# amankhullar/MMBiDAF

Measured on NVIDIA B200. Metric: mmbidaf_train_videos_per_s, higher is better.
Workload: dtype bf16 tcgen05 BiDAF + tf32 library GEMMs, fp32 accumulate / soft-max / LSTM

## Files before the change

### include/mmbidaf_b200.h

```cpp
#ifndef MMBIDAF_B200_H_
#define MMBIDAF_B200_H_

#include <stddef.h>
#include <stdint.h>

#ifdef __cplusplus
extern "C" {
#endif

#if defined(__GNUC__)
#define MMB_API __attribute__((visibility("default")))
#else
#define MMB_API
#endif

typedef void* mmb_stream_t;

enum mmb_status {
  MMB_OK = 0,
  MMB_ERR_INVALID = 1,
  MMB_ERR_UNSUPPORTED = 2,
  MMB_ERR_CUDA = 3
};

// ... 82 lines not shown
                                               const float* out_wt, const float* out_b, const float* emb_text, const float* h0,
                                               const uint8_t* mask, const int32_t* text_len, long long* tokens, int32_t* parents,
                                               float* scores, float* probs, long long* best, int32_t* path, int B, int Lt, int D, int H,
                                               int E, int M, int K, int S, int no_repeat, int min_sentences, mmb_stream_t stream);
MMB_API int mmb_decoder_beam_sample_fused(const float* proj_a, const float* proj_i, const float* enc_a, const float* enc_i,
                                          const float* Wh4t, const float* bh4, const float* v1, const float* wc1, const float* v2,
                                          const float* wc2, const float* v1b, const float* v2b, const float* Wb13t, const float* vb1,
                                          const float* vb2, const float* vb1b, const float* vb2b, const float* Wcatt, const float* bcat,
                                          const float* out_wt, const float* out_b, const float* emb_text, const float* h0,
                                          const uint8_t* mask, const int32_t* text_len, const unsigned long long* key, long long* tokens,
                                          int32_t* parents, float* scores, float* probs, float* phi, float* keys, long long* paths,
                                          int32_t* path_slots, float* kappa, int B, int Lt, int D, int H, int E, int M, int K, int S,
                                          float T, int no_repeat, int min_sentences, mmb_stream_t stream);
MMB_API int mmb_decoder_sample_fused(const float* proj_a, const float* proj_i, const float* enc_a, const float* enc_i,
                                     const float* Wh4t, const float* bh4, const float* v1, const float* wc1, const float* v2,
                                     const float* wc2, const float* v1b, const float* v2b, const float* Wb13t, const float* vb1,
                                     const float* vb2, const float* vb1b, const float* vb2b, const float* Wcatt, const float* bcat,
                                     const float* out_wt, const float* out_b, const float* emb_text, const float* h0,
                                     const uint8_t* mask, const int32_t* text_len, const unsigned long long* key, float* probs,
                                     long long* tokens, int B, int Lt, int D, int H, int E, int M, int S, int N, float T, int top_k,
                                     int no_repeat, int min_sentences, mmb_stream_t stream);
MMB_API int mmb_sample_pick(const float* probs, const uint8_t* eligible, const unsigned long long* key, const int32_t* row_base, int R,
                            int M, int S, int s, int N, float T, int top_k, long long* picks, mmb_stream_t stream);
MMB_API int mmb_decoder_sample_nucleus_fused(const float* proj_a, const float* proj_i, const float* enc_a, const float* enc_i,
                                             const float* Wh4t, const float* bh4, const float* v1, const float* wc1, const float* v2,
                                             const float* wc2, const float* v1b, const float* v2b, const float* Wb13t, const float* vb1,
                                             const float* vb2, const float* vb1b, const float* vb2b, const float* Wcatt, const float* bcat,
                                             const float* out_wt, const float* out_b, const float* emb_text, const float* h0,
                                             const uint8_t* mask, const int32_t* text_len, const unsigned long long* key, float* probs,
                                             long long* tokens, int B, int Lt, int D, int H, int E, int M, int S, int N, float T,
                                             int top_k, int no_repeat, int min_sentences, float top_p, mmb_stream_t stream);
MMB_API int mmb_sample_pick_nucleus(const float* probs, const uint8_t* eligible, const unsigned long long* key, const int32_t* row_base,
                                    int R, int M, int S, int s, int N, float T, int top_k, long long* picks, float top_p,
                                    mmb_stream_t stream);
MMB_API int mmb_greedy_select(const long long* argmax, const int32_t* text_len, int32_t* sel, int32_t* count, int B, int S,
                              mmb_stream_t stream);

MMB_API int mmb_decoder_attn_fwd(const float* proj_a, const float* proj_i, const float* enc_a, const float* enc_i,
                                 const float* hw, const float* coverage, const float* v1, const float* wc1,
                                 const float* v2, const float* wc2, const float* v1b, const float* v2b, float* p,
                                 float* stats, float* ctxp, float* ctx12, float* scale, int* counters, int B, int Lt, int D,
                                 int nch, mmb_stream_t stream);
MMB_API int mmb_decoder_attn_finish(const float* pb, const float* hw, const float* ctx12, const float* scale,
                                    const float* coverage, const float* sent, const float* h, const float* vb1,
                                    const float* vb2, const float* vb1b, const float* vb2b, float* p_alpha, float* xcat,
                                    float* att_cov, float* cov_out, float* beta, float* cov_loss, int B, int Lt, int D,
                                    int E, int H, int nch, mmb_stream_t stream);
MMB_API int mmb_decoder_cell_fwd(float* gates, const float* cell, float* h_out, float* cell_out, int B, int H,
                                 mmb_stream_t stream);
MMB_API int mmb_decoder_out_softmax(float* logits, const uint8_t* mask, long long* argmax, const long long* target,
                                    float* nll, int B, int M, mmb_stream_t stream);

MMB_API int mmb_decoder_bwd_head(const float* probs, const float* d_probs, const long long* target, const float* g_nll,
                                 const float* g_cov, const float* out_w, const float* gates, const float* cell_in,
                                 const float* cell_out, const float* d_h_out, const float* d_cell_out, const float* Wcat_ctx,
                                 const float* d_att_cov, const float* d_cov_out, const float* alpha, const float* beta,
                                 const float* ctx12, const float* pb, const float* hw, const float* vb1, const float* vb2,
                                 const float* att, const float* cov_out, const float* Wb13, float* d_logits, int ldd, float* d_gates,
                                 int ldg, float* d_cell, float* datt, float* dcov_tot, float* d_pre_b, float* d_ctx12, float* vec_acc,
                                 float* scal_acc, int B, int Lt, int D, int H, int M, mmb_stream_t stream);
MMB_API int mmb_decoder_out_softmax_bwd(const float* probs, const float* d_probs, const long long* target,
                                        const float* g_nll, float* d_logits, int ldd, int B, int M, mmb_stream_t stream);
MMB_API int mmb_decoder_cell_bwd(float* gates, const float* cell_in, const float* cell_out, const float* d_h,
                                 const float* d_h2, const float* d_cell_out, float* d_gates, int ldg, float* d_cell,
                                 int B, int H, mmb_stream_t stream);
MMB_API int mmb_decoder_attn_finish_bwd(const float* d_xcat, int ldx, const float* d_att_cov, const float* d_cov_out,
                                        const float* alpha, const float* beta, const float* ctx12, const float* pb,
                                        const float* hw, const float* vb1, const float* vb2, float* datt, float* d_pre_b,
                                        float* d_ctx12, float* vec_acc, float* scal_acc, const float* att_cov,
                                        const float* cov_out, const float* g_cov, float* dcov_tot, int B, int Lt, int D,
                                        mmb_stream_t stream);
MMB_API int mmb_decoder_step_fused_bwd(const float* probs, const float* d_probs, const long long* target, const float* g_nll,
                                       const float* g_cov, const float* out_w, const float* gates, const float* cell_in,
                                       const float* cell_out, const float* d_h_out, const float* d_cell_out, const float* Wcat_ctx,
                                       const float* d_att_cov, const float* d_cov_out, const float* alpha, const float* beta,
                                       const float* ctx12, const float* pb, const float* hw, const float* vb1, const float* vb2,
                                       const float* att, const float* cov_out, const float* Wb13, float* d_logits, int ldd,
                                       float* d_gates, int ldg, float* d_cell, float* datt, float* dcov_tot, float* d_pre_b,
                                       float* d_ctx12, float* vec_acc, float* scal_acc, const float* proj_a, const float* proj_i,
                                       const float* enc_a, const float* enc_i, const float* coverage, const float* v1, const float* wc1,
                                       const float* v2, const float* wc2, float* d_proj_a, float* d_proj_i, float* d_cov,
                                       const float* Wh_stack, float* d_h, int B, int Lt, int D, int H, int M, mmb_stream_t stream);

MMB_API int mmb_decoder_attn_bwd(const float* proj_a, const float* proj_i, const float* enc_a, const float* enc_i,
                                 const float* hw, const float* coverage, const float* alpha, const float* beta,
                                 const float* datt, const float* d_ctx12, const float* d_cov_out, const float* d_pre_b,
                                 const float* v1, const float* wc1, const float* v2, const float* wc2, float* d_alpha,
                                 float* spart, float* d_proj_a, float* d_proj_i, float* d_cov, float* colp, float* separt,
                                 float* d_hw4, int ldhw, float* vec_acc, float* scal_acc, int* counters, int B, int Lt,
                                 int D, int nch, mmb_stream_t stream);

MMB_API int mmb_masked_softmax_fwd(const float* x, const uint8_t* mask, float* y, long long rows, int n, int log_mode,
                                   mmb_stream_t stream);
MMB_API int mmb_masked_softmax_bwd(const float* y, const float* dy, const uint8_t* mask, float* dx, long long rows,
                                   int n, int log_mode, mmb_stream_t stream);

MMB_API int mmb_highway_fwd(const float* pre, const float* x, float* y, long long n, int H, mmb_stream_t stream);
MMB_API int mmb_highway_bwd(const float* pre, const float* x, const float* dy, float* d_pre, float* dx_direct,
                            long long n, int H, mmb_stream_t stream);

MMB_API int mmb_length_plan(const int32_t* lengths, uint8_t* mask, uint8_t* dec_mask, int32_t* order, int B, int L, int M,
                            mmb_stream_t stream);

MMB_API int mmb_col_sum_blocks(long long n, int p);
MMB_API int mmb_col_sum(const float* a, float* partial, float* out, long long n, int p, mmb_stream_t stream);

MMB_API int mmb_pack_segments(const float* const* srcs, const long long* dst_offsets, const long long* sizes, int n_segs, float* dst,
                              mmb_stream_t stream);

MMB_API int mmb_adadelta_clip_step(float* param, float* grad, float* square_avg, float* acc_delta, const float* grad_norm,
                                   float max_norm, float lr, float rho, float eps, float weight_decay, long long n,
                                   mmb_stream_t stream);

#ifdef __cplusplus
}
#endif
#endif
```

### mmbidaf_b200/_lib.py

```python
from __future__ import annotations

import ctypes
import os
from typing import Optional

import torch

_PKG = os.path.dirname(os.path.abspath(__file__))
LIB_PATH = os.path.join(_PKG, "libmmbidaf_b200.so")

_lib: Optional[ctypes.CDLL] = None
_device_ok = False

c_void_p, c_int, c_float, c_size_t = ctypes.c_void_p, ctypes.c_int, ctypes.c_float, ctypes.c_size_t

SIGNATURES = {
    "mmb_version": [],
    "mmb_last_error": [],
    "mmb_device_supported": [],
    "mmb_bidaf_fwd": [c_void_p] * 10 + [c_float] + [c_void_p] * 6 + [c_int] * 5 + [c_void_p],
    "mmb_bidaf_workspace_bytes": [c_int] * 6,
    "mmb_bidaf_bwd": [c_void_p] * 11 + [c_float] + [c_void_p] * 13 + [c_int] * 5 + [c_void_p],
    "mmb_bidaf_bwd_workspace_bytes": [c_int] * 5,
    "mmb_bilstm_fwd": [c_void_p] * 8 + [c_int] * 5 + [c_void_p],
    "mmb_bilstm_bwd": [c_void_p] * 8 + [c_int] * 4 + [c_void_p],
    "mmb_bilstm_fwd_dropout": [c_void_p] * 10 + [c_float] + [c_int] * 5 + [c_void_p],
    "mmb_bilstm_bwd_dropout": [c_void_p] * 9 + [c_float] + [c_int] * 4 + [c_void_p],
    "mmb_dropout_mask": [c_void_p, c_float, ctypes.c_longlong, c_void_p, c_void_p],
    "mmb_rng_next": [c_void_p, c_void_p, c_int, c_void_p],
    "mmb_dropout_apply": [c_void_p, c_void_p, c_void_p, c_float, ctypes.c_longlong, c_void_p],
    "mmb_decoder_chunks": [c_int, c_int],
    "mmb_decoder_step_fused_fwd": [c_void_p] * 42 + [c_int] * 6 + [c_void_p],
    "mmb_decoder_greedy_fused": [c_void_p] * 28 + [c_int] * 8 + [c_void_p],
    "mmb_decoder_beam_fused": [c_void_p] * 31 + [c_int] * 8 + [c_void_p],
    "mmb_decoder_greedy_constrained_fused": [c_void_p] * 27 + [c_int] * 9 + [c_void_p],
    "mmb_decoder_beam_constrained_fused": [c_void_p] * 31 + [c_int] * 10 + [c_void_p],
    "mmb_decoder_beam_sample_fused": [c_void_p] * 35 + [c_int] * 8 + [c_float] + [c_int] * 2 + [c_void_p],
    "mmb_decoder_sample_fused":[c_void_p] * 28 + [c_int] * 8 + [c_float] + [c_int] * 3 + [c_void_p],
    "mmb_sample_pick": [c_void_p] * 4 + [c_int] * 5 + [c_float, c_int, c_void_p, c_void_p],
    "mmb_decoder_sample_nucleus_fused": [c_void_p] * 28 + [c_int] * 8 + [c_float] + [c_int] * 3 + [c_float, c_void_p],
    "mmb_sample_pick_nucleus": [c_void_p] * 4 + [c_int] * 5 + [c_float, c_int, c_void_p, c_float, c_void_p],
    "mmb_greedy_select": [c_void_p] * 4 + [c_int] * 2 + [c_void_p],
    "mmb_decoder_bwd_head": [c_void_p] * 25 + [c_int] + [c_void_p] + [c_int] + [c_void_p] * 7 + [c_int] * 5 + [c_void_p],
    "mmb_decoder_attn_fwd": [c_void_p] * 18 + [c_int] * 4 + [c_void_p],
    "mmb_decoder_attn_finish": [c_void_p] * 17 + [c_int] * 6 + [c_void_p],
    "mmb_decoder_cell_fwd": [c_void_p] * 4 + [c_int] * 2 + [c_void_p],
    "mmb_decoder_out_softmax": [c_void_p] * 5 + [c_int] * 2 + [c_void_p],
    "mmb_decoder_out_softmax_bwd": [c_void_p] * 5 + [c_int] * 3 + [c_void_p],
    "mmb_decoder_cell_bwd": [c_void_p] * 7 + [c_int] + [c_void_p] + [c_int] * 2 + [c_void_p],
    "mmb_decoder_attn_finish_bwd": [c_void_p, c_int] + [c_void_p] * 18 + [c_int] * 3 + [c_void_p],
    "mmb_decoder_step_fused_bwd": [c_void_p] * 25 + [c_int] + [c_void_p] + [c_int] + [c_void_p] * 21 + [c_int] * 5 + [c_void_p],
    "mmb_decoder_attn_bwd": [c_void_p] * 24 + [c_int] + [c_void_p] * 3 + [c_int] * 4 + [c_void_p],
    "mmb_highway_fwd": [c_void_p] * 3 + [ctypes.c_longlong, c_int, c_void_p],
    "mmb_highway_bwd": [c_void_p] * 5 + [ctypes.c_longlong, c_int, c_void_p],
    "mmb_length_plan": [c_void_p] * 4 + [c_int] * 3 + [c_void_p],
    "mmb_pack_segments": [c_void_p] * 3 + [c_int] + [c_void_p] * 2,
    "mmb_col_sum_blocks": [ctypes.c_longlong, c_int],
    "mmb_col_sum": [c_void_p] * 3 + [ctypes.c_longlong, c_int, c_void_p],
    "mmb_adadelta_clip_step": [c_void_p] * 5 + [c_float] * 5 + [ctypes.c_longlong, c_void_p],
    "mmb_masked_softmax_fwd": [c_void_p] * 3 + [ctypes.c_longlong, c_int, c_int, c_void_p],
    "mmb_masked_softmax_bwd": [c_void_p] * 4 + [ctypes.c_longlong, c_int, c_int, c_void_p],
}
_RESTYPES = {"mmb_last_error": ctypes.c_char_p, "mmb_bidaf_workspace_bytes": c_size_t,
             "mmb_bidaf_bwd_workspace_bytes": c_size_t}


DECODER_WEIGHT_FIELDS = ("W2", "b2", "Wc1", "bc1", "v1", "v1b", "W4", "b4", "Wc2", "bc2", "v2", "v2b",
                         "Wb1", "bb1", "Wb2", "bb2", "Wb3", "bb3", "Wb4", "bb4", "vb1", "vb1b", "vb2", "vb2b",
                         "lstm_w_ih", "lstm_w_hh", "lstm_b_ih", "lstm_b_hh", "out_w", "out_b")


def load() -> ctypes.CDLL:
    global _lib
    if _lib is None:
        if not os.path.exists(LIB_PATH):
            raise RuntimeError(f"{LIB_PATH} is missing: run `python -m mmbidaf_b200.build` "
                               "(there is no CPU or PyTorch fallback for the mmbidaf_b200 kernels)")
        lib = ctypes.CDLL(LIB_PATH)
        for name, argtypes in SIGNATURES.items():
            fn = getattr(lib, name)
            fn.argtypes = argtypes
            fn.restype = _RESTYPES.get(name, c_int)
        _lib = lib
    return _lib


def lib() -> ctypes.CDLL:
    global _device_ok
    handle = load()
    if not _device_ok:
        if not torch.cuda.is_available():
            raise RuntimeError("mmbidaf_b200 needs a CUDA device (sm_100a); none is visible and there is no CPU path")
        if not handle.mmb_device_supported():
            raise RuntimeError(handle.mmb_last_error().decode())
        _device_ok = True
    return handle


def check(status: int, what: str) -> None:
    if status != 0:
        raise RuntimeError(f"{what} failed (status {status}): {load().mmb_last_error().decode()}")


def ptr(t: Optional[torch.Tensor]) -> Optional[int]:
    if t is None:
        return None
    assert t.is_cuda and t.is_contiguous(), "mmbidaf_b200 ops take contiguous CUDA tensors"
    return t.data_ptr()


def stream() -> int:
    return torch.cuda.current_stream().cuda_stream
```

### mmbidaf_b200/csrc/decoder_fused.cu

```cuda
#include <cooperative_groups.h>
#include <stdlib.h>
#include <type_traits>
#include "common.cuh"
#include "tc_common.cuh"

namespace cg = cooperative_groups;

namespace mmb {
namespace {

constexpr int NT = 512;
constexpr int NW = NT / 32;
constexpr int MAXC = 8;
constexpr int SCR = 2048;
__host__ __device__ constexpr int split4(int n, int parts) { return ((n + parts - 1) / parts + 3) & ~3; }

__device__ __forceinline__ float rcp_ftz(float x) {
  float y;
  asm("rcp.approx.ftz.f32 %0, %1;" : "=f"(y) : "f"(x));
  return y;
}

__device__ __forceinline__ void bulk_reduce_add_f32(float* dst, uint32_t src_smem, uint32_t bytes) {
  asm volatile("cp.reduce.async.bulk.global.shared::cta.bulk_group.add.f32 [%0], [%1], %2;" ::"l"(dst), "r"(src_smem), "r"(bytes)
// ... 252 lines not shown
      const float p = m < M ? v[m] : -1.f;
      const uint32_t bits = __float_as_uint(p);
      uint32_t q = __float2uint_rz(p * 16777216.f);
      const bool in = q != 0u && (bits & pmask) == prefix;
      const uint32_t digit = in ? (bits >> shift) & (kNucBuckets - 1) : kNucBuckets;
      q = in ? q : 0u;
      const uint32_t peers = __match_any_sync(0xffffffffu, digit);
      const uint32_t sum = __reduce_add_sync(peers, q);
      if (in && lane == __ffs(peers) - 1) atomicAdd(hist + digit, (unsigned long long)sum);
    }
    __syncthreads();
    const unsigned long long h = tid < kNucBuckets ? hist[kNucBuckets - 1 - tid] : 0ull;
    unsigned long long s = h;
#pragma unroll
    for (int o = 1; o < 32; o <<= 1) {
      const unsigned long long t = __shfl_up_sync(0xffffffffu, s, o);
      if (lane >= o) s += t;
    }
    if (lane == 31 && warp < kNucBuckets / 32) red[warp] = s;
    __syncthreads();
    unsigned long long below = 0, total = 0;
    for (int w = 0; w < kNucBuckets / 32; ++w) {
      below += w < warp ? red[w] : 0ull;
      total += red[w];
    }
    s += below;
    if (pass == 0) {
      const unsigned long long pq = (unsigned long long)P * total;
      rem = (pq >> 24) + ((pq & 0xffffffull) != 0ull);
      if (rem == 0ull) { first = true; break; }
    }
    if (tid < kNucBuckets && s - h < rem && rem <= s) {
      red[8] = (unsigned long long)(kNucBuckets - 1 - tid);
      red[9] = rem - (s - h);
    }
    __syncthreads();
    prefix |= (uint32_t)red[8] << shift;
    pmask |= (uint32_t)(kNucBuckets - 1) << shift;
    rem = red[9];
  }
  unsigned long long ties = 1;
  if (first) {
    uint32_t mx = 0;
    for (int m = tid; m < M; m += NT) {
      const float p = v[m];
      if (p >= 0.f) mx = max(mx, __float_as_uint(p));
    }
    mx = __reduce_max_sync(0xffffffffu, mx);
    __syncthreads();
    if (lane == 0) red[warp] = mx;
    __syncthreads();
    prefix = 0;
    for (int w = 0; w < NW; ++w) prefix = max(prefix, (uint32_t)red[w]);
  } else {
    const unsigned long long qs = __float2uint_rz(__uint_as_float(prefix) * 16777216.f);
    ties = (rem + qs - 1) / qs;
  }
  const int c = (M + NT - 1) / NT, lo = min(M, tid * c), hi = min(M, lo + c);
  int cnt = 0;
  for (int m = lo; m < hi; ++m) cnt += __float_as_uint(v[m]) == prefix;
  int incl = cnt;
#pragma unroll
  for (int o = 1; o < 32; o <<= 1) {
    const int t = __shfl_up_sync(0xffffffffu, incl, o);
    if (lane >= o) incl += t;
  }
  __syncthreads();
  if (lane == 31) red[warp] = (unsigned long long)incl;
  if (tid == 0) red[NW] = ~0ull;
  __syncthreads();
  unsigned long long excl = (unsigned long long)(incl - cnt);
  for (int w = 0; w < warp; ++w) excl += red[w];
  if (excl < ties && ties <= excl + (unsigned long long)cnt) {
    unsigned long long k = excl;
    for (int m = lo; m < hi; ++m)
      if (__float_as_uint(v[m]) == prefix && ++k == ties) red[NW] = (unsigned long long)m;
  }
  __syncthreads();
  const NucleusCut cut{prefix, (int)(long long)red[NW]};
  __syncthreads();
  return cut;
}

template <bool kGreedy, bool kBeam = false, bool kConstrained = false, bool kSample = false, bool kNucleus = false, bool kStoch = false>
__device__ __forceinline__ void dec_fused_body(const FusedArgs& a, const GreedyArgs& g, const BeamArgs& bm, const ConstraintArgs& cn,
                                               const SampleArgs sp, const NucleusArgs nu = NucleusArgs{}, const StochArgs st = StochArgs{}) {
  cg::cluster_group cluster = cg::this_cluster();
  const int CL = (int)cluster.num_blocks(), R = (int)cluster.block_rank();
  const int ob = blockIdx.x / CL;
  const int b = kSample ? cluster_row() / sp.N : ob;
  const int tid = threadIdx.x, lane = tid & 31, warp = tid >> 5;
  const int D = a.D, H = a.H, E = a.E, M = a.M, Lt = a.Lt, K = D + E + H;

  extern __shared__ __align__(16) float smem[];
  auto up4 = [](int v) { return (v + 3) & ~3; };
  float* s_hw = smem;
  float* s_x = s_hw + up4(4 * D);
  float* s_ctx = s_x + up4(K);
  float* s_pb = s_ctx + up4(2 * D);
  float* s_hn = s_pb + up4(2 * D);
  float* s_part = s_hn + up4(H);
  float* s_ex = s_part + up4(MAXC * (4 + 2 * D));
  float* s_g = s_ex + MAXC * 8;
  float* s_red = s_g + up4(4 * (split4(H, MAXC / 2) + 1));
  float* s_scr = s_red + 32;
  float* s_vec = s_scr + SCR;
  float* s_e = s_vec + up4(4 * D);
  float* s_cov = s_e + up4(2 * a.chunk);
  float* s_cpart = s_cov + up4(a.chunk);

  const int t0 = min(Lt, R * a.chunk), t1 = min(Lt, t0 + a.chunk), n = t1 - t0;
  const bool staged = a.stage_off != 0;
  float* const s_st0 = smem + a.stage_off + 4;
  float* const s_st1 = s_st0 + up4(a.chunk * D);
  const uint32_t bar_proj = tc::smem_u32(smem + a.stage_off), bar_enc = bar_proj + 8;
  const uint32_t stage_bytes = (uint32_t)(n * D) * 4u;
  if (staged && tid == 0) {
    tc::mbar_init(bar_proj, 1);
    tc::mbar_init(bar_enc, 1);
    tc::fence_barrier_init();
    if (n > 0) {
      tc::mbar_expect_tx(bar_proj, 2 * stage_bytes, 1);
      tc::tma_bulk_g2s(tc::smem_u32(s_st0), a.proj_a + ((size_t)b * Lt + t0) * D, stage_bytes, bar_proj, 1);
      tc::tma_bulk_g2s(tc::smem_u32(s_st1), a.proj_i + ((size_t)b * Lt + t0) * D, stage_bytes, bar_proj, 1);
    }
  }
  DEC_STAMP(0);
  const int S = kGreedy ? g.steps : 1;
  float cell_own = 0.f;
  int pick = 0;
  const int KW = kBeam ? bm.K : 1;
  const int ldh = up4(H), ldc = up4(split4(H, CL)), ldv = up4(a.chunk), ldp = up4((M + CL - 1) / CL);
  float* const bs_score = smem + (kSample ? sp.off : bm.off);
  int* const bs_tok = reinterpret_cast<int*>(bs_score + MAXK);
  int* const bs_stat = bs_tok + MAXK;
  float* const nt_score = bs_score + 3 * MAXK;
  int* const nt_tok = reinterpret_cast<int*>(nt_score + MAXK);
  int* const nt_par = nt_tok + MAXK;
  int* const nt_kind = nt_par + MAXK;
  constexpr int CS = kStoch ? MAXK + 1 : MAXK;
  float* const s_cand = nt_score + 4 * MAXK;
  float* const s_wred = s_cand + MAXC * CS * 4;
  float* const s_loc = s_wred + NW * 4;
  float* const s_bh = s_loc + CS * 4;
  float* const s_bhn = s_bh + KW * ldh;
  float* const s_bc = s_bhn + KW * ldh;
  float* const s_bcn = s_bc + KW * ldc;
  float* const s_bcv = s_bcn + KW * ldc;
  float* const s_bcvn = s_bcv + KW * ldv;
  float* const s_bp = s_bcvn + KW * ldv;
  const int eos = kBeam ? bm.text_len[b] - 1 : kConstrained ? cn.text_len[b] - 1 : 0;
  int runs = 0;
  const int e_per = (M + CL - 1) / CL, e_m0 = min(M, R * e_per), e_m1 = min(M, e_m0 + e_per);
  auto allowed0 = [&](int m) { return m < e_m1 && m <= eos && a.mask[(size_t)b * M + m] != 0; };
  const int ldu = (ldp + 31) / 32;
  uint32_t* bu_cur = reinterpret_cast<uint32_t*>(s_bp + KW * ldp);
  uint32_t* bu_nxt = bu_cur + KW * ldu;
  int* bk_cur = reinterpret_cast<int*>(bu_nxt + KW * ldu);
  int* bk_nxt = bk_cur + MAXK;
  uint32_t allow = 0;
  int kept = 0;
  uint32_t key0 = 0, key1 = 0;
  float inv_t = 1.f;
  if constexpr (kSample && !kConstrained) {
    const unsigned long long key = *sp.key;
    key0 = (uint32_t)key;
    key1 = (uint32_t)(key >> 32);
// ... 271 lines not shown
      block_matvec_t(a.Wb13t + (size_t)k * D * D, D, nullptr, s_ctx + k * D, D, hi - lo, s_scr, SCR, ((lo - k * D) & 3) == 0,
                     [&](int i) { return lo - k * D + i; },
                     [&](int i, float v) {
                       const int o = lo + i;
                       for (int r = 0; r < CL; ++r) cluster.map_shared_rank(s_pb, r)[o] = v;
                       if constexpr (!kGreedy) a.pb[((size_t)k * a.B + b) * D + (o - k * D)] = v;
                     });
    }
  }
  DEC_STAMP(9);
  cluster.sync();
  DEC_STAMP(10);
  float beta1, beta2;
  {
    float eb1 = 0.f, eb2 = 0.f;
    for (int d = tid; d < D; d += NT) {
      eb1 = fmaf(a.vb1[d], tanh_fast(s_pb[d] + s_hw[2 * D + d]), eb1);
      eb2 = fmaf(a.vb2[d], tanh_fast(s_pb[D + d] + s_hw[3 * D + d]), eb2);
    }
    eb1 = block_sum(eb1, s_red) + a.vb1b[0];
    eb2 = block_sum(eb2, s_red) + a.vb2b[0];
    const float mb = fmaxf(eb1, eb2);
    const float x1 = expf(eb1 - mb), x2 = expf(eb2 - mb);
    beta1 = x1 / (x1 + x2);
    beta2 = x2 / (x1 + x2);
    for (int d = tid; d < D; d += NT) s_x[d] = s_ctx[d] * beta1 + s_ctx[D + d] * beta2;
    float closs = 0.f;
    for (int i = tid; i < n; i += NT) {
      const int t = t0 + i;
      const float a1 = s_e[i] * scale_own[0], a2 = s_e[a.chunk + i] * scale_own[1];
      if constexpr (!kGreedy) {
        a.alpha[((size_t)b * 2 + 0) * Lt + t] = a1;
        a.alpha[((size_t)b * 2 + 1) * Lt + t] = a2;
      }
      const float att = a1 * beta1 + a2 * beta2;
      if constexpr (kBeam) {
        const float cnew = s_cov[i] + att;
        s_bcvn[slot * ldv + i] = cnew;
        closs += fminf(att, cnew);
      } else if constexpr (kGreedy) {
        const float cnew = s_cov[i] + att;
        s_cov[i] = cnew;
        closs += fminf(att, cnew);
      } else {
        const float cnew = a.cov[(size_t)b * Lt + t] + att;
        a.att_cov[(size_t)b * Lt + t] = att;
        a.cov_out[(size_t)b * Lt + t] = cnew;
        closs += fminf(att, cnew);
      }
    }
    closs = block_sum(closs, s_red);
    if (tid == 0) cluster.map_shared_rank(s_ex, 0)[R * 8 + 0] = closs;
    if (!kGreedy && R == 0 && tid == 0) {
      a.beta[b * 2 + 0] = beta1;
      a.beta[b * 2 + 1] = beta2;
    }
  }
  __syncthreads();
  if (!kGreedy && R == 0)
    for (int i = tid; i < K; i += NT) a.xcat[(size_t)b * K + i] = s_x[i];

  DEC_STAMP(11);
  {
    const int per = split4(H, CL), j0 = R * per, j1 = min(H, j0 + per), nj = max(0, j1 - j0);
    block_matvec_t(a.Wcatt, 4 * H, a.bcat, s_x, K, 4 * nj, s_scr, SCR, ((H | nj) & 3) == 0, [&](int i) { return (i / nj) * H + j0 + (i % nj); },
                   [&](int i, float v) { s_g[(i / nj) * (per + 1) + (i % nj)] = v; });
    __syncthreads();
    if (tid < nj) {
      const int j = j0 + tid;
      const float gi = gate_act(s_g[tid], 1.f), gf = gate_act(s_g[(per + 1) + tid], 1.f), gg = tanh_fast(s_g[2 * (per + 1) + tid]),
                  go = gate_act(s_g[3 * (per + 1) + tid], 1.f);
      const float c = fmaf(gf, kBeam ? s_bc[slot * ldc + tid] : kGreedy ? cell_own : a.cell[(size_t)b * H + j], gi * gg);
      const float hn = go * tanh_fast(c);
      if constexpr (kBeam) {
        s_bcn[slot * ldc + tid] = c;
      } else if constexpr (kGreedy) {
        cell_own = c;
      } else {
        a.cell_out[(size_t)b * H + j] = c;
        a.h_out[(size_t)b * H + j] = hn;
        float* gs = a.gates + (size_t)b * 4 * H;
        gs[j] = gi; gs[H + j] = gf; gs[2 * H + j] = gg; gs[3 * H + j] = go;
      }
      for (int r = 0; r < CL; ++r) cluster.map_shared_rank(s_hn, r)[j] = hn;
    }
  }
  DEC_STAMP(12);
  cluster.sync();
  DEC_STAMP(13);
  if constexpr (kBeam)
    for (int i = tid; i < H; i += NT) s_bhn[slot * ldh + i] = s_hn[i];
  const size_t prow = kGreedy ? (size_t)(kSample ? cluster_row() : ob) * S + s : (size_t)b;
  const int lrow = kGreedy ? s * 2 * a.B + b : b;
  if (R == 0 && tid == 0 && a.cov_loss) {
    float cs = 0.f;
    for (int r = 0; r < CL; ++r) cs += s_ex[r * 8 + 0];
    a.cov_loss[lrow] = cs;
  }

  {
    const int per = (M + CL - 1) / CL, m0 = min(M, R * per), m1 = min(M, m0 + per);
    float* const lg = s_cpart;
    block_matvec_t(a.out_wt, M, a.out_b, s_hn, H, m1 - m0, s_scr, SCR, (m0 & 3) == 0, [&](int i) { return m0 + i; }, [&](int i, float v) { lg[i] = v; });
    __syncthreads();
    for (int m = m0 + tid; m < m1; m += NT)
      if (!a.mask[(size_t)b * M + m]) lg[m - m0] = kNegFill;
    __syncthreads();
    float mx = -INFINITY;
    for (int m = m0 + tid; m < m1; m += NT) mx = fmaxf(mx, lg[m - m0]);
    mx = block_max(mx, s_red);
    float sum = 0.f;
    for (int m = m0 + tid; m < m1; m += NT) sum += expf(lg[m - m0] - mx);
    sum = block_sum(sum, s_red);
    if (tid < CL) {
      float* dst = cluster.map_shared_rank(s_ex, tid) + R * 8;
      dst[1] = mx;
      dst[2] = sum;
    }
    DEC_STAMP(14);
    cluster.sync();
    DEC_STAMP(15);
    float gmx = -INFINITY;
    for (int r = 0; r < CL; ++r)
      if (min(M, r * per) < M) gmx = fmaxf(gmx, s_ex[r * 8 + 1]);
    float gsum = 0.f;
    for (int r = 0; r < CL; ++r)
      if (min(M, r * per) < M) gsum = fmaf(s_ex[r * 8 + 2], expf(s_ex[r * 8 + 1] - gmx), gsum);
    const float inv = 1.f / gsum;
    float best = -INFINITY;
    int best_i = M;
    const int tg = a.target ? (int)a.target[kGreedy ? b * g.T + s : b] : -1;
    const bool eos_ok = kConstrained && !kBeam && eos_allowed(cn, eos, kept);
    const uint32_t cbase = ((uint32_t)(kSample ? cluster_row() : 0) * (uint32_t)S + (uint32_t)s) * (uint32_t)M;
    for (int m = m0 + tid; m < m1; m += NT) {
      const float p = expf(lg[m - m0] - gmx) * inv;
      if constexpr (kBeam) s_bp[slot * ldp + m - m0] = p;
      else a.probs[prow * M + m] = p;
      if constexpr (kSample) {
        const bool cand = !kConstrained || (((allow >> ((unsigned)(m - m0) / NT)) & 1u) && (m != eos || eos_ok));
        if (sp.top_k > 0) {
          lg[m - m0] = p;
        } else if constexpr (kNucleus) {
          for (int r = 0; r < CL; ++r) cluster.map_shared_rank(smem + nu.off, r)[m] = cand ? p : -1.f;
        } else if (cand) {
          const float z = kConstrained ? sample_z(sp, p, cbase + (uint32_t)m) : sample_score(p, inv_t, cbase + (uint32_t)m, key0, key1);
          if (z > best || best_i == M) { best = z; best_i = m; }
        }
      } else if constexpr (kConstrained && !kBeam) {
        if (((allow >> ((unsigned)(m - m0) / NT)) & 1u) && (m != eos || eos_ok) && p > best) { best = p; best_i = m; }
      } else if (p > best) { best = p; best_i = m; }
      if (m == tg && a.nll) a.nll[lrow] = -logf(p + 1e-12f);
    }
    if constexpr (kNucleus) {
      if (sp.top_k == 0) {
        cluster.sync();
        const float* const nv = smem + nu.off;
        const NucleusCut cut = nucleus_cut(nv, M, nu.P, reinterpret_cast<unsigned long long*>(smem + nu.off + up4(M)),
                                           reinterpret_cast<unsigned long long*>(smem + nu.off + up4(M) + 2 * kNucBuckets));
        for (int m = m0 + tid; m < m1; m += NT) {
          const float p = nv[m];
          const uint32_t bits = __float_as_uint(p);
          if (p >= 0.f && (bits > cut.pstar || (bits == cut.pstar && m <= cut.mstar))) {
            const float z = kConstrained ? sample_z(sp, p, cbase + (uint32_t)m) : sample_score(p, inv_t, cbase + (uint32_t)m, key0, key1);
            if (z > best || best_i == M) { best = z; best_i = m; }
          }
        }
      }
    }
    if (!kBeam && (kGreedy || a.argmax) && !(kSample && sp.top_k > 0)) {
      const float bbest = block_max(best, s_red);
      int cand = best == bbest ? best_i : M;
#pragma unroll
      for (int o = 16; o > 0; o >>= 1) cand = min(cand, __shfl_xor_sync(0xffffffffu, cand, o));
      __shared__ int redi[NW];
      __syncthreads();
      if (lane == 0) redi[warp] = cand;
      __syncthreads();
      if (tid == 0) {
        int r = M;
        for (int w = 0; w < NW; ++w) r = min(r, redi[w]);
        for (int q = 0; q < (kGreedy ? CL : 1); ++q) {
          float* dst = cluster.map_shared_rank(s_ex, q) + R * 8;
          dst[3] = bbest;
// ... 273 lines not shown
        if (R == 0 && tid == 0) a.argmax[(size_t)cluster_row() * S + s] = gi;
        pick = gi;
      }
    } else {
    __syncthreads();
    const size_t row = ((size_t)b * S + s) * KW;
    if (R == 0 && tid == 0)
      for (int j = 0; j < KW; ++j) {
        bm.tokens[row + j] = nt_tok[j];
        bm.parents[row + j] = nt_par[j];
        bm.scores[row + j] = nt_score[j];
        if constexpr (kStoch) {
          st.phi[row + j] = x_nphi[j];
          st.keys[row + j] = x_nkey[j];
        }
      }
    for (int i = tid; i < KW * nm; i += NT) {
      const int j = i / nm, m = m0 + (i - j * nm), kd = nt_kind[j];
      bm.probs[(row + j) * M + m] = (kd == 1 || kd == 2) ? s_bp[nt_par[j] * ldp + m - m0] : 0.f;
    }
    for (int j = 0; j < KW; ++j) {
      if (nt_kind[j] != 1) continue;
      const int q = nt_par[j];
      for (int i = tid; i < H; i += NT) s_bh[j * ldh + i] = s_bhn[q * ldh + i];
      for (int i = tid; i < ldc; i += NT) s_bc[j * ldc + i] = s_bcn[q * ldc + i];
      for (int i = tid; i < n; i += NT) s_bcv[j * ldv + i] = s_bcvn[q * ldv + i];
      if constexpr (kConstrained) {
        const int tk = nt_tok[j], rel = tk - m0;
        const bool clear = cn.no_repeat && tk < eos && rel >= 0 && tk < m1;
        for (int w = tid; w < ldu; w += NT)
          bu_nxt[j * ldu + w] = bu_cur[q * ldu + w] & ~(clear && (rel >> 5) == w ? 1u << (rel & 31) : 0u);
        if (tid == 0) bk_nxt[j] = bk_cur[q] + (tk < eos ? 1 : 0);
      }
    }
    if (tid < KW) {
      const int kd = nt_kind[tid];
      bs_score[tid] = nt_score[tid];
      bs_tok[tid] = nt_tok[tid];
      bs_stat[tid] = kd == 1 ? kLive : kd == 0 ? kEmpty : kDone;
      if constexpr (kStoch) {
        x_phi[tid] = x_nphi[tid];
        x_key[tid] = x_nkey[tid];
      }
    }
    __syncthreads();
    if constexpr (kConstrained) {
      uint32_t* const t = bu_cur; bu_cur = bu_nxt; bu_nxt = t;
      int* const u = bk_cur; bk_cur = bk_nxt; bk_nxt = u;
    }
    }
  }
  }
  if constexpr (kBeam) {
    if (staged && tid == 0 && n > 0) tc::mbar_wait(bar_proj, (uint32_t)(runs & 1));
    if constexpr (kStoch) {
      if (R == 0 && tid < KW) {
        const size_t o = ((size_t)b * KW + tid) * S;
        int j = bm.parents[((size_t)b * S + S - 1) * KW + tid] < 0 ? -1 : tid;
        for (int s = S - 1; s >= 0; --s) {
          const size_t row = ((size_t)b * S + s) * KW;
          st.path_slots[o + s] = j;
          st.paths[o + s] = j >= 0 ? bm.tokens[row + j] : eos;
          j = j >= 0 ? bm.parents[row + j] : -1;
        }
      }
    } else if (R == 0 && tid == 0) {
      int j = 0;
      for (int s = S - 1; s >= 0; --s) {
        const size_t row = ((size_t)b * S + s) * KW;
        bm.path[(size_t)b * S + s] = j;
        bm.best[(size_t)b * S + s] = j >= 0 ? bm.tokens[row + j] : -1;
        j = j >= 0 ? bm.parents[row + j] : -1;
      }
    }
  }
  DEC_STAMP(16);
  DEC_STAMP(17);
}

__global__ void __launch_bounds__(NT) dec_step_fused_kernel(const FusedArgs a) {
  dec_fused_body<false>(a, GreedyArgs{}, BeamArgs{}, ConstraintArgs{}, SampleArgs{});
}

__global__ void __launch_bounds__(NT) dec_greedy_fused_kernel(const FusedArgs a, const GreedyArgs g) {
  dec_fused_body<true>(a, g, BeamArgs{}, ConstraintArgs{}, SampleArgs{});
}

__global__ void __launch_bounds__(NT) dec_beam_fused_kernel(const FusedArgs a, const GreedyArgs g, const BeamArgs bm) {
  dec_fused_body<true, true>(a, g, bm, ConstraintArgs{}, SampleArgs{});
}

__global__ void __launch_bounds__(NT) dec_greedy_constrained_kernel(const FusedArgs a, const GreedyArgs g, const ConstraintArgs cn) {
  dec_fused_body<true, false, true>(a, g, BeamArgs{}, cn, SampleArgs{});
}

__global__ void __launch_bounds__(NT) dec_beam_constrained_kernel(const FusedArgs a, const GreedyArgs g, const BeamArgs bm,
                                                                  const ConstraintArgs cn) {
  dec_fused_body<true, true, true>(a, g, bm, cn, SampleArgs{});
}

__global__ void __launch_bounds__(NT) dec_sample_kernel(const FusedArgs a, const GreedyArgs g, const SampleArgs sp) {
  dec_fused_body<true, false, false, true>(a, g, BeamArgs{}, ConstraintArgs{}, sp);
}

__global__ void __launch_bounds__(NT) dec_sample_constrained_kernel(const FusedArgs a, const GreedyArgs g, const ConstraintArgs cn,
                                                                    const SampleArgs sp) {
  dec_fused_body<true, false, true, true>(a, g, BeamArgs{}, cn, sp);
}

__global__ void __launch_bounds__(NT) dec_sample_nucleus_kernel(const FusedArgs a, const GreedyArgs g, const SampleArgs sp,
                                                                const NucleusArgs nu) {
  dec_fused_body<true, false, false, true, true>(a, g, BeamArgs{}, ConstraintArgs{}, sp, nu);
}

__global__ void __launch_bounds__(NT) dec_sample_nucleus_constrained_kernel(const FusedArgs a, const GreedyArgs g,
                                                                            const ConstraintArgs cn, const SampleArgs sp,
                                                                            const NucleusArgs nu) {
  dec_fused_body<true, false, true, true, true>(a, g, BeamArgs{}, cn, sp, nu);
}

__global__ void __launch_bounds__(NT) dec_beam_sample_kernel(const FusedArgs a, const GreedyArgs g, const BeamArgs bm,
                                                             const StochArgs st) {
  dec_fused_body<true, true, false, false, false, true>(a, g, bm, ConstraintArgs{}, SampleArgs{}, NucleusArgs{}, st);
}

__global__ void __launch_bounds__(NT) dec_beam_sample_constrained_kernel(const FusedArgs a, const GreedyArgs g, const BeamArgs bm,
                                                                         const ConstraintArgs cn, const StochArgs st) {
  dec_fused_body<true, true, true, false, false, true>(a, g, bm, cn, SampleArgs{}, NucleusArgs{}, st);
}

}

struct HeadArgs {
  const float *probs, *d_probs;
  const long long* target;
  const float *g_nll, *g_cov;
  const float* out_w;
  const float *gates, *cell_in, *cell_out;
  const float *d_h_out, *d_cell_out;
  const float* Wcat_ctx;
  const float *d_att_cov, *d_cov_out;
  const float *alpha, *beta, *ctx12, *pb, *hw;
  const float *vb1, *vb2;
  const float *att, *cov_out;
  const float* Wb13;
  float* d_logits;
  float* d_gates;
  float *d_cell, *datt, *dcov_tot, *d_pre_b, *d_ctx12;
  float *vec_acc, *scal_acc;
  int B, Lt, D, H, M, ldd, ldg, chunk;
  int sweeps;
  const float *proj_a, *proj_i, *enc_a, *enc_i, *cov;
  const float *v1, *wc1, *v2, *wc2;
  float *d_proj_a, *d_proj_i, *d_cov;
  const float* Wh_stack;
  float* d_h;
  int stage_off;
};

__global__ void __launch_bounds__(NT) dec_bwd_head_kernel(const HeadArgs a) {
  cg::cluster_group cluster = cg::this_cluster();
  const int CL = (int)cluster.num_blocks(), R = (int)cluster.block_rank();
  const int b = blockIdx.x / CL;
  const int tid = threadIdx.x;
  const int D = a.D, H = a.H, M = a.M, Lt = a.Lt;

  extern __shared__ __align__(16) float smem[];
  auto up4 = [](int v) { return (v + 3) & ~3; };
  float* s_dl = smem;
  const int per_m = (M + CL - 1) / CL;
  float* s_dhp = s_dl + up4(per_m);
  float* s_dg = s_dhp + up4(MAXC * H);
  float* s_dctx = s_dg + up4(4 * H);
  float* s_dpre = s_dctx + up4(D);
  float* s_ex = s_dpre + up4(2 * D);
  float* s_red = s_ex + MAXC * 4;
  float* s_scr = s_red + 32;
  const int mv_cap = a.sweeps ? (a.stage_off != 0 ? NW / 2 : NW) * 3 * D : NT;
  float* const mv_scr = a.sweeps ? s_scr + NT + up4(2 * D) + up4(2 * a.chunk) + up4(4 * a.chunk) + up4(6 * D) : s_scr;
  const bool mv_quads = a.sweeps != 0;

  const int t0 = min(Lt, R * a.chunk), t1 = min(Lt, t0 + a.chunk), n = t1 - t0;
  const bool staged = a.stage_off != 0;
  float* const s_st0 = smem + a.stage_off + 4;
  float* const s_st1 = s_st0 + up4(a.chunk * D);
  const uint32_t bar_enc = tc::smem_u32(smem + a.stage_off), bar_proj = bar_enc + 8;
  const uint32_t stage_bytes = (uint32_t)(n * D) * 4u;
  if (staged && tid == 0) {
    tc::mbar_init(bar_enc, 1);
    tc::mbar_init(bar_proj, 1);
    tc::fence_barrier_init();
    if (n > 0) {
      tc::mbar_expect_tx(bar_enc, 2 * stage_bytes, 1);
      tc::tma_bulk_g2s(tc::smem_u32(s_st0), a.enc_a + ((size_t)b * Lt + t0) * D, stage_bytes, bar_enc, 1);
      tc::tma_bulk_g2s(tc::smem_u32(s_st1), a.enc_i + ((size_t)b * Lt + t0) * D, stage_bytes, bar_enc, 1);
    }
  }
  DEC_STAMP(18);
  const int m0 = min(M, R * per_m), m1 = min(M, m0 + per_m);
  const int tg = a.target ? (int)a.target[b] : -1;
  const float dp_t = a.target ? -a.g_nll[b] / (a.probs[(size_t)b * M + tg] + 1e-12f) : 0.f;
  if (a.d_probs) {
    float dot = 0.f;
    for (int m = m0 + tid; m < m1; m += NT) dot = fmaf(a.probs[(size_t)b * M + m], a.d_probs[(size_t)b * M + m], dot);
    dot = block_sum(dot, s_red);
    if (tid < CL) cluster.map_shared_rank(s_ex, tid)[R * 4 + 0] = dot;
    cluster.sync();
  }
  {
    float dot = 0.f;
    if (a.d_probs)
      for (int r = 0; r < CL; ++r) dot += s_ex[r * 4 + 0];
    if (a.target) dot = fmaf(a.probs[(size_t)b * M + tg], dp_t, dot);
    for (int m = m0 + tid; m < m1; m += NT) {
      const float dp = (a.d_probs ? a.d_probs[(size_t)b * M + m] : 0.f) + (m == tg ? dp_t : 0.f);
      const float v = a.probs[(size_t)b * M + m] * (dp - dot);
      s_dl[m - m0] = v;
      a.d_logits[(size_t)b * a.ldd + m] = v;
    }
    if (R == 0)
      for (int m = M + tid; m < a.ldd; m += NT) a.d_logits[(size_t)b * a.ldd + m] = 0.f;
  }
  __syncthreads();
  DEC_STAMP(19);
  block_matvec_t(a.out_w + (size_t)m0 * H, H, nullptr, s_dl, m1 - m0, H, mv_scr, mv_cap, mv_quads, [](int i) { return i; }, [&](int i, float v) {
    for (int r = 0; r < CL; ++r) cluster.map_shared_rank(s_dhp, r)[R * H + i] = v;
  });
  if (m1 - m0 <= 0 && tid < H)
    for (int r = 0; r < CL; ++r) cluster.map_shared_rank(s_dhp, r)[R * H + tid] = 0.f;
  cluster.sync();
  DEC_STAMP(20);
  if (tid < H) {
    const int j = tid;
    float dh = 0.f;
    for (int r = 0; r < CL; ++r) dh += s_dhp[r * H + j];
    if (a.d_h_out) dh += a.d_h_out[(size_t)b * H + j];
    const float* g = a.gates + (size_t)b * 4 * H;
    const float gi = g[j], gf = g[H + j], gg = g[2 * H + j], go = g[3 * H + j];
    const float tc = tanh_fast(a.cell_out[(size_t)b * H + j]);
    const float dc = fmaf(dh * go, 1.f - tc * tc, a.d_cell_out ? a.d_cell_out[(size_t)b * H + j] : 0.f);
    const float di = dc * gg * gi * (1.f - gi), df = dc * a.cell_in[(size_t)b * H + j] * gf * (1.f - gf);
    const float dg = dc * gi * (1.f - gg * gg), dO = dh * tc * go * (1.f - go);
    s_dg[j] = di; s_dg[H + j] = df; s_dg[2 * H + j] = dg; s_dg[3 * H + j] = dO;
    if (R == 0) {
      float* o = a.d_gates + (size_t)b * a.ldg;
      o[j] = di; o[H + j] = df; o[2 * H + j] = dg; o[3 * H + j] = dO;
      a.d_cell[(size_t)b * H + j] = dc * gf;
    }
  }
  __syncthreads();
  DEC_STAMP(21);
  {
    const int per = split4(D, CL), d0 = min(D, R * per), d1 = min(D, d0 + per);
    block_matvec_t(a.Wcat_ctx, D, nullptr, s_dg, 4 * H, d1 - d0, mv_scr, mv_cap, mv_quads, [&](int i) { return d0 + i; }, [&](int i, float v) {
      for (int r = 0; r < CL; ++r) cluster.map_shared_rank(s_dctx, r)[d0 + i] = v;
    });
  }
  cluster.sync();
  DEC_STAMP(22);
  const float beta1 = a.beta[b * 2 + 0], beta2 = a.beta[b * 2 + 1];
  {
    float db1 = 0.f, db2 = 0.f;
    if (R == 0)
      for (int d = tid; d < D; d += NT) {
        db1 = fmaf(a.ctx12[(size_t)b * D + d], s_dctx[d], db1);
        db2 = fmaf(a.ctx12[((size_t)a.B + b) * D + d], s_dctx[d], db2);
      }
    const float gc = a.g_cov ? a.g_cov[b] : 0.f;
    const int t0 = min(Lt, R * a.chunk), t1 = min(Lt, t0 + a.chunk);
    for (int t = t0 + tid; t < t1; t += NT) {
      float dcv = a.d_cov_out ? a.d_cov_out[(size_t)b * Lt + t] : 0.f;
      float g = a.d_att_cov ? a.d_att_cov[(size_t)b * Lt + t] : 0.f;
      if (a.g_cov) {
        const float av = a.att[(size_t)b * Lt + t], cv = a.cov_out[(size_t)b * Lt + t];
        const float tie = av == cv ? 0.5f * gc : 0.f;
        g += av < cv ? gc : tie;
        dcv += cv < av ? gc : tie;
      }
      a.dcov_tot[(size_t)b * Lt + t] = dcv;
      g += dcv;
      a.datt[(size_t)b * Lt + t] = g;
      db1 = fmaf(a.alpha[((size_t)b * 2 + 0) * Lt + t], g, db1);
      db2 = fmaf(a.alpha[((size_t)b * 2 + 1) * Lt + t], g, db2);
    }
    db1 = block_sum(db1, s_red);
    db2 = block_sum(db2, s_red);
    if (tid < CL) {
      float* dst = cluster.map_shared_rank(s_ex, tid) + R * 4;
      dst[1] = db1;
      dst[2] = db2;
    }
  }
  cluster.sync();
  {
    float db1 = 0.f, db2 = 0.f;
    for (int r = 0; r < CL; ++r) {
      db1 += s_ex[r * 4 + 1];
      db2 += s_ex[r * 4 + 2];
    }
    const float mix = beta1 * db1 + beta2 * db2;
    const float deb1 = beta1 * (db1 - mix), deb2 = beta2 * (db2 - mix);
    for (int d = tid; d < D; d += NT) {
      const float t1 = tanh_fast(a.pb[(size_t)b * D + d] + a.hw[(size_t)b * 4 * D + 2 * D + d]);
      const float t2 = tanh_fast(a.pb[((size_t)a.B + b) * D + d] + a.hw[(size_t)b * 4 * D + 3 * D + d]);
      const float p1 = deb1 * a.vb1[d] * (1.f - t1 * t1), p2 = deb2 * a.vb2[d] * (1.f - t2 * t2);
      s_dpre[d] = p1;
      s_dpre[D + d] = p2;
      if (R == 0) {
        a.d_pre_b[(size_t)b * D + d] = p1;
        a.d_pre_b[((size_t)a.B + b) * D + d] = p2;
        a.vec_acc[((size_t)b * 6 + 4) * D + d] += deb1 * t1;
        a.vec_acc[((size_t)b * 6 + 5) * D + d] += deb2 * t2;
      }
    }
    if (R == 0 && tid == 0) {
      a.scal_acc[b * 4 + 2] += deb1;
      a.scal_acc[b * 4 + 3] += deb2;
    }
// ... 198 lines not shown
    }
    float xacc[2] = {0.f, 0.f};
    for (int w0 = 0; w0 < NW; w0 += PW) {
      if (warp >= w0 && warp < w0 + PW) {
#pragma unroll
        for (int j = 0; j < NJ; ++j) {
          const int d = lane + 32 * j;
          if (d < D) {
            s_part[((warp - w0) * 3 + 0) * D + d] = c_dz[j];
            s_part[((warp - w0) * 3 + 1) * D + d] = c_cov[j];
            s_part[((warp - w0) * 3 + 2) * D + d] = c_v[j];
          }
        }
      }
      __syncthreads();
#pragma unroll
      for (int q = 0; q < 2; ++q) {
        const int i = tid + q * NT;
        if (i < 3 * D)
          for (int w = 0; w < PW; ++w) xacc[q] += s_part[w * 3 * D + i];
      }
      __syncthreads();
    }
#pragma unroll
    for (int q = 0; q < 2; ++q) {
      const int i = tid + q * NT;
      if (i < 3 * D)
        for (int r = 0; r < CL; ++r) cluster.map_shared_rank(s_colp, r)[(R * 2 + m) * 3 * D + i] = xacc[q];
    }
  };
  if (staged && n > 0) tc::mbar_wait(bar_proj, 0);
  for (int m = 0; m < 2; ++m) {
    if (staged) {
      float* const sp = m == 0 ? s_st0 : s_st1;
      if (nj7) sweep8(m, sp, N7{}, std::true_type{}); else sweep8(m, sp, N8{}, std::true_type{});
    } else {
      float* const gp = const_cast<float*>(m == 0 ? a.proj_a : a.proj_i) + ((size_t)b * Lt + t0) * D;
      if (nj7) sweep8(m, gp, N7{}, std::false_type{}); else sweep8(m, gp, N8{}, std::false_type{});
    }
  }
  for (int i = tid; i < n; i += NT) a.d_cov[(size_t)b * Lt + t0 + i] = s_row[i];
  if (tid < CL) {
    float* dst = cluster.map_shared_rank(s_ex, tid) + R * 4;
    dst[2] = se_m0;
    dst[3] = se_m1;
  }
  cluster.sync();
  DEC_STAMP(26);
  for (int i = tid; i < 2 * D; i += NT) {
    const int m = i / D, d = i - m * D;
    float x = 0.f, y = 0.f, z = 0.f;
    for (int r = 0; r < CL; ++r) {
      const float* q = s_colp + (r * 2 + m) * 3 * D;
      x += q[d];
      y += q[D + d];
      z += q[2 * D + d];
    }
    s_in[4 * H + m * D + d] = x;
    s_in[4 * H + (2 + m) * D + d] = s_dpre[m * D + d];
    if (R == 0) {
      float* o = a.d_gates + (size_t)b * a.ldg + 4 * H;
      o[m * D + d] = x;
      o[(2 + m) * D + d] = s_dpre[m * D + d];
      a.vec_acc[((size_t)b * 6 + m) * D + d] += y;
      a.vec_acc[((size_t)b * 6 + 2 + m) * D + d] += z;
    }
  }
  for (int i = tid; i < 4 * H; i += NT) s_in[i] = s_dg[i];
  if (R == 0 && tid < 2) {
    float sv = 0.f;
    for (int r = 0; r < CL; ++r) sv += s_ex[r * 4 + 2 + tid];
    a.scal_acc[b * 4 + tid] += sv;
  }
  __syncthreads();
  {
    const int per = split4(H, CL), j0 = min(H, R * per), j1 = min(H, j0 + per);
    block_matvec_t(a.Wh_stack, H, nullptr, s_in, 4 * H + 4 * D, j1 - j0, mv_scr, mv_cap, mv_quads, [&](int i) { return j0 + i; },
                   [&](int i, float v) { a.d_h[(size_t)b * H + j0 + i] = v; });
  }
  if (staged && tid == 0) bulk_wait_all();
  DEC_STAMP(27);
}

static size_t g_head_smem_set = 0;

static size_t head_smem_bytes(int D, int H, int M, int CL, int chunk = 0, bool sweeps = false, int PW = NW) {
  auto up4 = [](size_t v) { return (v + 3) & ~(size_t)3; };
  const size_t per_m = (M + CL - 1) / CL;
  size_t floats = up4(per_m) + up4((size_t)MAXC * H) + up4(4 * H) + up4(D) + up4(2 * D) + MAXC * 4 + 32 + NT;
  if (sweeps)
    floats += up4(2 * D) + up4(2 * (size_t)chunk) + up4(4 * (size_t)chunk) + up4(6 * D) + up4((size_t)PW * 3 * D) + up4(chunk) + up4((size_t)CL * 6 * D) +
              up4(4 * H + 4 * D);
  return floats * sizeof(float) + 64;
}

static size_t fused_smem_bytes(int Lt, int D, int H, int E, int M, int CL, int* chunk_out) {
  const int chunk = (Lt + CL - 1) / CL;
  const int K = D + E + H;
  const int groups = (D & 3) == 0 ? NT / (D >> 2) : NT / D;
  const int per_m = (M + CL - 1) / CL;
  int cpart = groups * 2 * D;
  if (cpart < per_m) cpart = per_m;
  auto up4 = [](size_t v) { return (v + 3) & ~(size_t)3; };
  const size_t floats = up4(4 * D) + up4(K) + 2 * up4(2 * D) + up4(H) + up4((size_t)MAXC * (4 + 2 * D)) + MAXC * 8 +
                        up4(4 * (split4(H, MAXC / 2) + 1)) + 32 + SCR + up4(4 * D) + up4(2 * (size_t)chunk) + up4(chunk) + up4(cpart);
  if (chunk_out) *chunk_out = chunk;
  return floats * sizeof(float) + 64;
}

static size_t beam_floats(int K, int CL, int chunk, int H, int M, bool constrained = false) {
  auto up4 = [](size_t v) { return (v + 3) & ~(size_t)3; };
  const size_t ldp = up4((M + CL - 1) / CL);
  const size_t per_slot = 2 * (up4(H) + up4(split4(H, CL)) + up4(chunk)) + ldp;
  const size_t cons = constrained ? 2 * (size_t)K * ((ldp + 31) / 32) + 2 * MAXK : 0;
  return 7 * MAXK + MAXC * MAXK * 4 + NW * 4 + MAXK * 4 + (size_t)K * per_slot + cons;
}

static size_t nucleus_floats(int M) { return (((size_t)M + 3) & ~(size_t)3) + 2 * kNucBuckets + 2 * 32; }

constexpr size_t kStochBeamExtra = MAXC * 4 + 4;
static size_t stoch_floats(int K, int CL, int M) {
  const size_t ldp = (((size_t)M + CL - 1) / CL + 3) & ~(size_t)3;
  return 5 * MAXK + 2 * MAXC * MAXK + 2 * MAXC * MAXK + (size_t)K * ldp;
}

static int launch_fused(FusedArgs a, const GreedyArgs* g, const char* who, mmb_stream_t stream, BeamArgs* bm = nullptr,
                        const ConstraintArgs* cn = nullptr, SampleArgs* sp = nullptr, NucleusArgs* nu = nullptr,
                        StochArgs* sb = nullptr) {
  const int B = a.B, Lt = a.Lt, D = a.D, H = a.H, E = a.E, M = a.M;
  MMB_REQUIRE(B > 0 && Lt > 0 && D > 0 && H > 0 && E >= 0 && M > 0, MMB_ERR_INVALID,
              "%s: B=%d Lt=%d D=%d H=%d E=%d M=%d", who, B, Lt, D, H, E, M);
  MMB_REQUIRE(D <= 256, MMB_ERR_UNSUPPORTED, "%s: D=%d > 256", who, D);
  const int rows = sp ? B * sp->N : B;
  const int CL = (long long)rows * 4 * 2 <= 160 ? 8 : 4;
  size_t smem = fused_smem_bytes(Lt, D, H, E, M, CL, &a.chunk);
  MMB_REQUIRE(smem <= 200 * 1024, MMB_ERR_UNSUPPORTED, "%s: %zu B of shared memory (Lt=%d)", who, smem, Lt);
  MMB_REQUIRE(!cn || bm || (M + CL - 1) / CL <= 32 * NT, MMB_ERR_UNSUPPORTED, "%s: M=%d > %d sentences per CTA", who, M, 32 * NT);
  if (bm) {
    bm->off = (int)((smem + 15) / 16 * 4);
    smem = ((size_t)bm->off + beam_floats(bm->K, CL, a.chunk, H, M, cn != nullptr)) * 4 + 64;
    if (sb) {
      sb->off = (int)(((size_t)bm->off + beam_floats(bm->K, CL, a.chunk, H, M, cn != nullptr) + kStochBeamExtra + 3) & ~(size_t)3);
      smem = ((size_t)sb->off + stoch_floats(bm->K, CL, M)) * 4 + 64;
    }
    MMB_REQUIRE(smem <= 227 * 1024, MMB_ERR_UNSUPPORTED, "%s: width %d needs %zu B of shared memory per CTA, more than 232448 (B=%d Lt=%d M=%d)",
                who, bm->K, smem, B, Lt, M);
  } else if (sp) {
    sp->off = (int)((smem + 15) / 16 * 4);
    smem = ((size_t)sp->off + beam_floats(0, CL, a.chunk, H, M)) * 4 + 64;
    if (nu) {
      nu->off = (int)((smem + 15) / 16 * 4);
      smem = ((size_t)nu->off + nucleus_floats(M)) * 4 + 64;
      MMB_REQUIRE(smem <= 227 * 1024, MMB_ERR_UNSUPPORTED, "%s: the nucleus row of M=%d needs %zu B of shared memory per CTA, more than "
                  "232448 (Lt=%d)", who, M, smem, Lt);
    }
  }
  {
    static const char* stage_env = getenv("MMB_DEC_STAGE");
    const size_t base_floats = (smem + 15) / 16 * 4;
    const size_t stage_floats = 4 + 2 * (((size_t)a.chunk * D + 3) & ~(size_t)3);
    const bool enc_aligned = ((reinterpret_cast<uintptr_t>(a.enc_a) | reinterpret_cast<uintptr_t>(a.enc_i)) & 15) == 0;
    const bool aligned = enc_aligned && ((reinterpret_cast<uintptr_t>(a.proj_a) | reinterpret_cast<uintptr_t>(a.proj_i)) & 15) == 0;
    a.ctx_vec4 = (D & 3) == 0 && enc_aligned;
    if ((D & 3) == 0 && aligned && (base_floats + stage_floats) * 4 <= 227 * 1024 && !(stage_env && atoi(stage_env) == 0)) {
      a.stage_off = (int)base_floats;
      smem = (base_floats + stage_floats) * 4;
    }
  }
  static size_t smem_set[11] = {0, 0, 0, 0, 0, 0, 0, 0, 0, 0, 0};
  const int which = sb ? (cn ? 10 : 9) : nu ? (cn ? 8 : 7) : sp ? (cn ? 6 : 5) : bm ? (cn ? 4 : 2) : g ? (cn ? 3 : 1) : 0;
  if (smem > smem_set[which]) {
    const void* fn = which == 10 ? (const void*)dec_beam_sample_constrained_kernel : which == 9 ? (const void*)dec_beam_sample_kernel
                   : which == 8 ? (const void*)dec_sample_nucleus_constrained_kernel : which == 7 ? (const void*)dec_sample_nucleus_kernel
                   : which == 6 ? (const void*)dec_sample_constrained_kernel : which == 5 ? (const void*)dec_sample_kernel
                   : which == 4 ? (const void*)dec_beam_constrained_kernel : which == 3 ? (const void*)dec_greedy_constrained_kernel
                   : which == 2 ? (const void*)dec_beam_fused_kernel : which == 1 ? (const void*)dec_greedy_fused_kernel
                                : (const void*)dec_step_fused_kernel;
    MMB_CUDA(cudaFuncSetAttribute(fn, cudaFuncAttributeMaxDynamicSharedMemorySize, (int)smem));
    smem_set[which] = smem;
  }
  static const char* trace_env = getenv("MMB_DEC_TRACE");
  static bool trace_set = false;
  if (trace_env && !trace_set) {
    long long* ptr = reinterpret_cast<long long*>(strtoull(trace_env, nullptr, 0));
    MMB_CUDA(cudaMemcpyToSymbol(g_dec_trace, &ptr, sizeof(ptr)));
    trace_set = true;
  }
  cudaLaunchConfig_t cfg{};
  cfg.gridDim = dim3((unsigned)(rows * CL));
  cfg.blockDim = dim3(NT);
  cfg.dynamicSmemBytes = smem;
  cfg.stream = static_cast<cudaStream_t>(stream);
  cudaLaunchAttribute attr[1];
  attr[0].id = cudaLaunchAttributeClusterDimension;
  attr[0].val.clusterDim.x = (unsigned)CL;
  attr[0].val.clusterDim.y = 1;
  attr[0].val.clusterDim.z = 1;
  cfg.attrs = attr;
  cfg.numAttrs = 1;
  if (sb && cn) {
    MMB_CUDA(cudaLaunchKernelEx(&cfg, dec_beam_sample_constrained_kernel, a, *g, *bm, *cn, *sb));
    return check_launch("dec_beam_sample_constrained_kernel");
  }
  if (sb) {
    MMB_CUDA(cudaLaunchKernelEx(&cfg, dec_beam_sample_kernel, a, *g, *bm, *sb));
    return check_launch("dec_beam_sample_kernel");
  }
  if (nu && cn) {
    MMB_CUDA(cudaLaunchKernelEx(&cfg, dec_sample_nucleus_constrained_kernel, a, *g, *cn, *sp, *nu));
    return check_launch("dec_sample_nucleus_constrained_kernel");
  }
  if (nu) {
    MMB_CUDA(cudaLaunchKernelEx(&cfg, dec_sample_nucleus_kernel, a, *g, *sp, *nu));
    return check_launch("dec_sample_nucleus_kernel");
  }
  if (sp && cn) {
    MMB_CUDA(cudaLaunchKernelEx(&cfg, dec_sample_constrained_kernel, a, *g, *cn, *sp));
    return check_launch("dec_sample_constrained_kernel");
  }
  if (sp) {
    MMB_CUDA(cudaLaunchKernelEx(&cfg, dec_sample_kernel, a, *g, *sp));
    return check_launch("dec_sample_kernel");
  }
  if (cn && bm) {
    MMB_CUDA(cudaLaunchKernelEx(&cfg, dec_beam_constrained_kernel, a, *g, *bm, *cn));
    return check_launch("dec_beam_constrained_kernel");
  }
  if (cn) {
    MMB_CUDA(cudaLaunchKernelEx(&cfg, dec_greedy_constrained_kernel, a, *g, *cn));
    return check_launch("dec_greedy_constrained_kernel");
  }
  if (bm) {
    MMB_CUDA(cudaLaunchKernelEx(&cfg, dec_beam_fused_kernel, a, *g, *bm));
    return check_launch("dec_beam_fused_kernel");
  }
  if (g) {
    MMB_CUDA(cudaLaunchKernelEx(&cfg, dec_greedy_fused_kernel, a, *g));
    return check_launch("dec_greedy_fused_kernel");
  }
  MMB_CUDA(cudaLaunchKernelEx(&cfg, dec_step_fused_kernel, a));
  return check_launch("dec_step_fused_kernel");
}

}

extern "C" int mmb_decoder_step_fused_fwd(const float* proj_a, const float* proj_i, const float* enc_a, const float* enc_i,
                                          const float* Wh4t, const float* bh4, const float* v1, const float* wc1, const float* v2,
                                          const float* wc2, const float* v1b, const float* v2b, const float* Wb13t, const float* vb1,
                                          const float* vb2, const float* vb1b, const float* vb2b, const float* Wcatt,
                                          const float* bcat, const float* out_wt, const float* out_b, const float* sent,
                                          const float* h, const float* cell, const float* cov, const uint8_t* mask,
                                          const long long* target, float* probs, float* h_out, float* cell_out, float* att_cov,
                                          float* cov_out, long long* argmax, float* nll, float* cov_loss, float* hw, float* alpha,
                                          float* beta, float* ctx12, float* pb, float* xcat, float* gates, int B, int Lt, int D,
                                          int H, int E, int M, mmb_stream_t stream) {
  using namespace mmb;
  MMB_REQUIRE(proj_a && proj_i && enc_a && enc_i && Wh4t && bh4 && v1 && wc1 && v2 && wc2 && v1b && v2b && Wb13t && vb1 && vb2 &&
                  vb1b && vb2b && Wcatt && bcat && out_wt && out_b && sent && h && cell && cov && mask && probs && h_out &&
                  cell_out && att_cov && cov_out && hw && alpha && beta && ctx12 && pb && xcat && gates,
              MMB_ERR_INVALID, "mmb_decoder_step_fused_fwd: null pointer");
  FusedArgs a{proj_a, proj_i, enc_a, enc_i, Wh4t, bh4, v1, wc1, v2, wc2, v1b, v2b, Wb13t, vb1, vb2, vb1b, vb2b, Wcatt, bcat, out_wt, out_b,
              sent, h, cell, cov, mask, target, probs, h_out, cell_out, att_cov, cov_out, argmax, nll, cov_loss, hw, alpha, beta,
              ctx12, pb, xcat, gates, B, Lt, D, H, E, M, 0, 0};
  return launch_fused(a, nullptr, "mmb_decoder_step_fused_fwd", stream);
}

extern "C" int mmb_decoder_greedy_fused(const float* proj_a, const float* proj_i, const float* enc_a, const float* enc_i,
                                        const float* Wh4t, const float* bh4, const float* v1, const float* wc1, const float* v2,
                                        const float* wc2, const float* v1b, const float* v2b, const float* Wb13t, const float* vb1,
                                        const float* vb2, const float* vb1b, const float* vb2b, const float* Wcatt, const float* bcat,
                                        const float* out_wt, const float* out_b, const float* emb_text, const float* h0,
                                        const uint8_t* mask, const long long* target, float* probs, long long* argmax,
                                        float* loss_terms, int B, int Lt, int D, int H, int E, int M, int S, int T,
                                        mmb_stream_t stream) {
  using namespace mmb;
  MMB_REQUIRE(proj_a && proj_i && enc_a && enc_i && Wh4t && bh4 && v1 && wc1 && v2 && wc2 && v1b && v2b && Wb13t && vb1 && vb2 &&
                  vb1b && vb2b && Wcatt && bcat && out_wt && out_b && emb_text && h0 && mask && probs && argmax,
              MMB_ERR_INVALID, "mmb_decoder_greedy_fused: null pointer");
  MMB_REQUIRE(S > 0 && (!target || (loss_terms && T >= S)), MMB_ERR_INVALID, "mmb_decoder_greedy_fused: S=%d T=%d, target %s, loss_terms %s",
              S, T, target ? "set" : "null", loss_terms ? "set" : "null");
  FusedArgs a{proj_a, proj_i, enc_a, enc_i, Wh4t, bh4, v1, wc1, v2, wc2, v1b, v2b, Wb13t, vb1, vb2, vb1b, vb2b, Wcatt, bcat, out_wt, out_b,
              nullptr, nullptr, nullptr, nullptr, mask, target, probs, nullptr, nullptr, nullptr, nullptr, argmax,
// ... 131 lines not shown
  FusedArgs a{proj_a, proj_i, enc_a, enc_i, Wh4t, bh4, v1, wc1, v2, wc2, v1b, v2b, Wb13t, vb1, vb2, vb1b, vb2b, Wcatt, bcat, out_wt, out_b,
              nullptr, nullptr, nullptr, nullptr, mask, nullptr, probs, nullptr, nullptr, nullptr, nullptr, tokens,
              nullptr, nullptr, nullptr, nullptr, nullptr, nullptr, nullptr, nullptr, nullptr, B, Lt, D, H, E, M, 0, 0};
  const GreedyArgs g{emb_text, h0, S, 0};
  const ConstraintArgs cn{text_len, no_repeat, min_sentences};
  SampleArgs sp{key, T, N, top_k, 0};
  return launch_fused(a, &g, who, stream, nullptr, constrained ? &cn : nullptr, &sp, nu);
}
}

extern "C" int mmb_decoder_sample_fused(const float* proj_a, const float* proj_i, const float* enc_a, const float* enc_i,
                                        const float* Wh4t, const float* bh4, const float* v1, const float* wc1, const float* v2,
                                        const float* wc2, const float* v1b, const float* v2b, const float* Wb13t, const float* vb1,
                                        const float* vb2, const float* vb1b, const float* vb2b, const float* Wcatt, const float* bcat,
                                        const float* out_wt, const float* out_b, const float* emb_text, const float* h0,
                                        const uint8_t* mask, const int* text_len, const unsigned long long* key, float* probs,
                                        long long* tokens, int B, int Lt, int D, int H, int E, int M, int S, int N, float T,
                                        int top_k, int no_repeat, int min_sentences, mmb_stream_t stream) {
  return mmb::sample_fused(proj_a, proj_i, enc_a, enc_i, Wh4t, bh4, v1, wc1, v2, wc2, v1b, v2b, Wb13t, vb1, vb2, vb1b, vb2b, Wcatt,
                           bcat, out_wt, out_b, emb_text, h0, mask, text_len, key, probs, tokens, B, Lt, D, H, E, M, S, N, T, top_k,
                           no_repeat, min_sentences, stream, nullptr, "mmb_decoder_sample_fused");
}

extern "C" int mmb_decoder_sample_nucleus_fused(const float* proj_a, const float* proj_i, const float* enc_a, const float* enc_i,
                                                const float* Wh4t, const float* bh4, const float* v1, const float* wc1, const float* v2,
                                                const float* wc2, const float* v1b, const float* v2b, const float* Wb13t, const float* vb1,
                                                const float* vb2, const float* vb1b, const float* vb2b, const float* Wcatt, const float* bcat,
                                                const float* out_wt, const float* out_b, const float* emb_text, const float* h0,
                                                const uint8_t* mask, const int* text_len, const unsigned long long* key, float* probs,
                                                long long* tokens, int B, int Lt, int D, int H, int E, int M, int S, int N, float T,
                                                int top_k, int no_repeat, int min_sentences, float top_p,
                                                mmb_stream_t stream) {
  using namespace mmb;
  MMB_REQUIRE(top_p > 0.f && top_p <= 1.f, MMB_ERR_INVALID, "mmb_decoder_sample_nucleus_fused: top_p=%g (in (0, 1])", (double)top_p);
  MMB_REQUIRE(top_p == 1.f || M < 65536, MMB_ERR_UNSUPPORTED, "mmb_decoder_sample_nucleus_fused: M=%d (below 65536 with top_p < 1)", M);
  NucleusArgs nu{(uint32_t)rintf(top_p * 16777216.f), 0};
  return sample_fused(proj_a, proj_i, enc_a, enc_i, Wh4t, bh4, v1, wc1, v2, wc2, v1b, v2b, Wb13t, vb1, vb2, vb1b, vb2b, Wcatt, bcat,
                      out_wt, out_b, emb_text, h0, mask, text_len, key, probs, tokens, B, Lt, D, H, E, M, S, N, T, top_k, no_repeat,
                      min_sentences, stream, top_p == 1.f ? nullptr : &nu, "mmb_decoder_sample_nucleus_fused");
}

extern "C" int mmb_decoder_bwd_head(const float* probs, const float* d_probs, const long long* target, const float* g_nll,
                                    const float* g_cov, const float* out_w, const float* gates, const float* cell_in,
                                    const float* cell_out, const float* d_h_out, const float* d_cell_out, const float* Wcat_ctx,
                                    const float* d_att_cov, const float* d_cov_out, const float* alpha, const float* beta,
                                    const float* ctx12, const float* pb, const float* hw, const float* vb1, const float* vb2,
                                    const float* att, const float* cov_out, const float* Wb13, float* d_logits, int ldd, float* d_gates,
                                    int ldg, float* d_cell, float* datt, float* dcov_tot, float* d_pre_b, float* d_ctx12, float* vec_acc,
                                    float* scal_acc, int B, int Lt, int D, int H, int M, mmb_stream_t stream) {
  using namespace mmb;
  MMB_REQUIRE(probs && out_w && gates && cell_in && cell_out && Wcat_ctx && alpha && beta && ctx12 && pb && hw && vb1 && vb2 && Wb13 &&
                  d_logits && d_gates && d_cell && datt && dcov_tot && d_pre_b && d_ctx12 && vec_acc && scal_acc,
              MMB_ERR_INVALID, "mmb_decoder_bwd_head: null pointer");
  MMB_REQUIRE((!target || g_nll) && (!g_cov || (att && cov_out)), MMB_ERR_INVALID, "mmb_decoder_bwd_head: loss-term pointers");
  MMB_REQUIRE(B > 0 && Lt > 0 && D > 0 && H > 0 && M > 0 && ldd >= M && ldg >= 4 * H && H <= NT, MMB_ERR_INVALID,
              "mmb_decoder_bwd_head: B=%d Lt=%d D=%d H=%d M=%d ldd=%d ldg=%d", B, Lt, D, H, M, ldd, ldg);
  const int CL = (long long)B * 4 * 2 <= 160 ? 8 : 4;
  HeadArgs a{probs, d_probs, target, g_nll, g_cov, out_w, gates, cell_in, cell_out, d_h_out, d_cell_out, Wcat_ctx, d_att_cov, d_cov_out,
             alpha, beta, ctx12, pb, hw, vb1, vb2, att, cov_out, Wb13, d_logits, d_gates, d_cell, datt, dcov_tot, d_pre_b, d_ctx12,
             vec_acc, scal_acc, B, Lt, D, H, M, ldd, ldg, (Lt + CL - 1) / CL,
             0, nullptr, nullptr, nullptr, nullptr, nullptr, nullptr, nullptr, nullptr, nullptr, nullptr, nullptr, nullptr, nullptr, nullptr, 0};
  const size_t smem = head_smem_bytes(D, H, M, CL);
  MMB_REQUIRE(smem <= 200 * 1024, MMB_ERR_UNSUPPORTED, "mmb_decoder_bwd_head: %zu B of shared memory", smem);
  if (smem > g_head_smem_set) {
    MMB_CUDA(cudaFuncSetAttribute(dec_bwd_head_kernel, cudaFuncAttributeMaxDynamicSharedMemorySize, (int)smem));
    g_head_smem_set = smem;
  }
  cudaLaunchConfig_t cfg{};
  cfg.gridDim = dim3((unsigned)(B * CL));
  cfg.blockDim = dim3(NT);
  cfg.dynamicSmemBytes = smem;
  cfg.stream = static_cast<cudaStream_t>(stream);
  cudaLaunchAttribute attr[1];
  attr[0].id = cudaLaunchAttributeClusterDimension;
  attr[0].val.clusterDim.x = (unsigned)CL;
  attr[0].val.clusterDim.y = 1;
  attr[0].val.clusterDim.z = 1;
  cfg.attrs = attr;
  cfg.numAttrs = 1;
  MMB_CUDA(cudaLaunchKernelEx(&cfg, dec_bwd_head_kernel, a));
  return check_launch("dec_bwd_head_kernel");
}

extern "C" int mmb_decoder_step_fused_bwd(const float* probs, const float* d_probs, const long long* target, const float* g_nll,
                                          const float* g_cov, const float* out_w, const float* gates, const float* cell_in,
                                          const float* cell_out, const float* d_h_out, const float* d_cell_out, const float* Wcat_ctx,
                                          const float* d_att_cov, const float* d_cov_out, const float* alpha, const float* beta,
                                          const float* ctx12, const float* pb, const float* hw, const float* vb1, const float* vb2,
                                          const float* att, const float* cov_out, const float* Wb13, float* d_logits, int ldd,
                                          float* d_gates, int ldg, float* d_cell, float* datt, float* dcov_tot, float* d_pre_b,
                                          float* d_ctx12, float* vec_acc, float* scal_acc, const float* proj_a, const float* proj_i,
                                          const float* enc_a, const float* enc_i, const float* coverage, const float* v1, const float* wc1,
                                          const float* v2, const float* wc2, float* d_proj_a, float* d_proj_i, float* d_cov,
                                          const float* Wh_stack, float* d_h, int B, int Lt, int D, int H, int M, mmb_stream_t stream) {
  using namespace mmb;
  MMB_REQUIRE(probs && out_w && gates && cell_in && cell_out && Wcat_ctx && alpha && beta && ctx12 && pb && hw && vb1 && vb2 && Wb13 &&
                  d_logits && d_gates && d_cell && datt && dcov_tot && d_pre_b && d_ctx12 && vec_acc && scal_acc && proj_a && proj_i &&
                  enc_a && enc_i && coverage && v1 && wc1 && v2 && wc2 && d_proj_a && d_proj_i && d_cov && Wh_stack && d_h,
              MMB_ERR_INVALID, "mmb_decoder_step_fused_bwd: null pointer");
  MMB_REQUIRE((!target || g_nll) && (!g_cov || (att && cov_out)), MMB_ERR_INVALID, "mmb_decoder_step_fused_bwd: loss-term pointers");
  MMB_REQUIRE(B > 0 && Lt > 0 && D > 0 && D <= 256 && H > 0 && M > 0 && ldd >= M && ldg >= 4 * H + 4 * D && H <= NT, MMB_ERR_INVALID,
              "mmb_decoder_step_fused_bwd: B=%d Lt=%d D=%d H=%d M=%d ldd=%d ldg=%d", B, Lt, D, H, M, ldd, ldg);
  const int CL = (long long)B * 4 * 2 <= 160 ? 8 : 4;
  const int chunk = (Lt + CL - 1) / CL;
  HeadArgs a{probs, d_probs, target, g_nll, g_cov, out_w, gates, cell_in, cell_out, d_h_out, d_cell_out, Wcat_ctx, d_att_cov, d_cov_out,
             alpha, beta, ctx12, pb, hw, vb1, vb2, att, cov_out, Wb13, d_logits, d_gates, d_cell, datt, dcov_tot, d_pre_b, d_ctx12,
             vec_acc, scal_acc, B, Lt, D, H, M, ldd, ldg, chunk,
             1, proj_a, proj_i, enc_a, enc_i, coverage, v1, wc1, v2, wc2, d_proj_a, d_proj_i, d_cov, Wh_stack, d_h, 0};
  size_t smem = head_smem_bytes(D, H, M, CL, chunk, true);
  MMB_REQUIRE(smem <= 200 * 1024, MMB_ERR_UNSUPPORTED, "mmb_decoder_step_fused_bwd: %zu B of shared memory (Lt=%d)", smem, Lt);
  {
    static const char* stage_env = getenv("MMB_DEC_STAGE");
    const size_t base_floats = (head_smem_bytes(D, H, M, CL, chunk, true, NW / 2) - 64) / 4;
    const size_t stage_floats = 4 + 2 * (((size_t)chunk * D + 3) & ~(size_t)3);
    const bool aligned = ((reinterpret_cast<uintptr_t>(proj_a) | reinterpret_cast<uintptr_t>(proj_i) | reinterpret_cast<uintptr_t>(enc_a) |
                           reinterpret_cast<uintptr_t>(enc_i) | reinterpret_cast<uintptr_t>(d_proj_a) |
                           reinterpret_cast<uintptr_t>(d_proj_i)) & 15) == 0;
    if ((D & 3) == 0 && aligned && (base_floats + stage_floats) * 4 + 64 <= 227 * 1024 && !(stage_env && atoi(stage_env) == 0)) {
      a.stage_off = (int)base_floats;
      smem = (base_floats + stage_floats) * 4 + 64;
    }
  }
  if (smem > g_head_smem_set) {
    MMB_CUDA(cudaFuncSetAttribute(dec_bwd_head_kernel, cudaFuncAttributeMaxDynamicSharedMemorySize, (int)smem));
    g_head_smem_set = smem;
  }
  cudaLaunchConfig_t cfg{};
  cfg.gridDim = dim3((unsigned)(B * CL));
  cfg.blockDim = dim3(NT);
  cfg.dynamicSmemBytes = smem;
  cfg.stream = static_cast<cudaStream_t>(stream);
  cudaLaunchAttribute attr[1];
  attr[0].id = cudaLaunchAttributeClusterDimension;
  attr[0].val.clusterDim.x = (unsigned)CL;
  attr[0].val.clusterDim.y = 1;
  attr[0].val.clusterDim.z = 1;
  cfg.attrs = attr;
  cfg.numAttrs = 1;
  MMB_CUDA(cudaLaunchKernelEx(&cfg, dec_bwd_head_kernel, a));
  return check_launch("dec_bwd_head_kernel (whole step)");
}
```

### mmbidaf_b200/functional.py

```python
from __future__ import annotations

import contextlib
from typing import Optional, Tuple

import torch

from . import ops


class _Lanes:
    enabled = False
    n = 4
    streams = {}
    used = set()
    rr = 0


@contextlib.contextmanager
def leaf_lanes():
    if not torch.cuda.is_available() or _Lanes.enabled:
        yield
        return
    _Lanes.enabled = True
    _Lanes.used = set()
# ... 287 lines not shown
        s = tape.seq
        B, D, H, E = s.B, s.D, s.H, s.E
        alpha = torch.stack(r["alpha"], dim=0)
        dctx12 = torch.stack(r["dctx12"], dim=0)
        d_enc_a = torch.bmm(alpha[:, :, 0].permute(1, 2, 0), dctx12[:, 0].permute(1, 0, 2))
        d_enc_i = torch.bmm(alpha[:, :, 1].permute(1, 2, 0), dctx12[:, 1].permute(1, 0, 2))
        with _leaf(tape.vec_acc, tape.scal_acc, *(t for k in ("h_prev", "xcat", "h_out", "dlog", "da", "dhw4", "dpre", "ctx12")
                                                    for t in r[k])):
            grads = _DecoderOpen._param_grads(ctx, tape, r, s)
        for v in r.values():
            v.clear()
        d_proj_a, d_proj_i = tape.d_proj_a, tape.d_proj_i
        tape.d_proj_a = tape.d_proj_i = tape.vec_acc = tape.scal_acc = None
        return (None, d_proj_a, d_proj_i, d_enc_a, d_enc_i, *grads)

    @staticmethod
    def _param_grads(ctx, tape, r, s):
        B, D, H, E = s.B, s.D, s.H, s.E
        cat = lambda k: torch.cat(r[k], dim=0)
        h_prev, xcat, h_out, dlog, da, dhw4 = cat("h_prev"), cat("xcat"), cat("h_out"), cat("dlog"), cat("da"), cat("dhw4")
        S = len(r["dlog"])
        kmajor = lambda k: torch.stack(r[k], dim=0).permute(1, 0, 2, 3).reshape(2, S * B, D)
        dpre, ctx12 = kmajor("dpre"), kmajor("ctx12")
        vec, scal = tape.vec_acc.sum(dim=0), tape.scal_acc.sum(dim=0)
        d_wh4 = dhw4.t() @ h_prev
        hw_sum = dhw4.sum(dim=0)
        d_wb13 = torch.bmm(dpre.transpose(1, 2), ctx12)
        pre_sum = dpre.sum(dim=1)
        d_wcat = da.t() @ xcat
        gate_sum = da.sum(dim=0)
        g = {
            "W2": d_wh4[:D], "b2": hw_sum[:D], "Wc1": vec[0].reshape(D, 1), "bc1": hw_sum[:D],
            "v1": vec[2].reshape(1, D), "v1b": scal[0:1],
            "W4": d_wh4[D:2 * D], "b4": hw_sum[D:2 * D], "Wc2": vec[1].reshape(D, 1), "bc2": hw_sum[D:2 * D],
            "v2": vec[3].reshape(1, D), "v2b": scal[1:2],
            "Wb1": d_wb13[0], "bb1": pre_sum[0], "Wb2": d_wh4[2 * D:3 * D], "bb2": hw_sum[2 * D:3 * D],
            "Wb3": d_wb13[1], "bb3": pre_sum[1], "Wb4": d_wh4[3 * D:], "bb4": hw_sum[3 * D:],
            "vb1": vec[4].reshape(1, D), "vb1b": scal[2:3], "vb2": vec[5].reshape(1, D), "vb2b": scal[3:4],
            "lstm_w_ih": d_wcat[:, :D + E], "lstm_w_hh": d_wcat[:, D + E:], "lstm_b_ih": gate_sum, "lstm_b_hh": gate_sum,
            "out_w": dlog.t() @ h_out, "out_b": dlog.sum(dim=0),
        }
        from ._lib import DECODER_WEIGHT_FIELDS
        return [g[name].reshape(shape) for name, shape in zip(DECODER_WEIGHT_FIELDS, ctx.shapes)]


class _DecoderStep(torch.autograd.Function):

    @staticmethod
    def forward(ctx, tape, token, sent, h, cell, cov, mask_u8, target):
        probs, h_out, cell_out, att, cov_out, _, saved, lossvec = ops.decoder_step_fwd(
            tape.seq, sent, h, cell, cov, mask_u8, target=target)
        ctx.tape = tape
        ctx.has_token = token is not None
        ctx.fused = target is not None
        extra = (target, att, cov_out) if ctx.fused else ()
        ctx.save_for_backward(h, cell, cov, probs, h_out, cell_out, *saved, *extra)
        ctx.set_materialize_grads(False)
        if lossvec is None:
            lossvec = probs.new_zeros(0)
        return probs, h_out, cell_out, att, cov_out, lossvec

    @staticmethod
    def backward(ctx, d_probs, d_h_out, d_cell_out, d_att, d_cov_out, d_lossvec):
        tape = ctx.tape
        if getattr(tape, "closed", False) or getattr(ctx, "consumed", False):
            raise RuntimeError("mmbidaf_b200: a decoder step's backward ran twice over one forward (retain_graph=True is not supported)")
        ctx.consumed = True
        h, cell, cov, probs, h_out, cell_out, *rest = ctx.saved_tensors
        saved, extra = rest[:7], rest[7:]
        target, att, cov_new = extra if ctx.fused else (None, None, None)
        tape.open_accumulators()
        d_h, d_cell, d_cov, d_logits, d_gates, d_ctx12, d_hw4, d_pre_b = ops.decoder_step_bwd(
            tape.seq, h, cell, cov, probs, cell_out, saved, d_probs, d_h_out, d_cell_out, d_att, d_cov_out,
            tape.d_proj_a, tape.d_proj_i, tape.vec_acc, tape.scal_acc,
            target=target if d_lossvec is not None else None, d_lossvec=d_lossvec, att_cov=att, cov_out=cov_new)
        hw, alpha, beta, ctx12, pb, xcat, gates = saved
        r = tape.rows
        r["h_prev"].append(h); r["xcat"].append(xcat); r["h_out"].append(h_out); r["alpha"].append(alpha)
        r["dlog"].append(d_logits); r["da"].append(d_gates); r["dctx12"].append(d_ctx12); r["dhw4"].append(d_hw4)
        r["dpre"].append(d_pre_b); r["ctx12"].append(ctx12)
        return None, (tape.zero_token(d_h) if ctx.has_token else None), None, d_h, d_cell, d_cov, None, None


class _DecodeLoss(torch.autograd.Function):

    _coef = {}

    _weights = {}

    @staticmethod
    def forward(ctx, steps, cov_weight, every_step, *terms):
        t = torch.stack(terms)
        S, _, B = t.shape
        ctx.meta = (S, steps, cov_weight, every_step, B)
        key = (t.device, t.dtype, S, steps, cov_weight, every_step, B)
        wvec = _DecodeLoss._weights.get(key)
        if wvec is None:
            w3 = torch.zeros(S, 2, B, dtype=t.dtype)
            w3[:, 0] = 1.0 / steps
            if every_step:
                w3[:, 1] = cov_weight / steps
            else:
                w3[-1, 1] = cov_weight / steps
            wvec = _DecodeLoss._weights[key] = w3.reshape(-1).to(t.device)
        return torch.dot(t.reshape(-1), wvec)

    @staticmethod
    def backward(ctx, g):
        S, steps, w, every_step, B = ctx.meta
        key = (g.device, steps, w, B)
        coef = _DecodeLoss._coef.get(key)
        if coef is None:
            coef = _DecodeLoss._coef[key] = torch.tensor([[1.0 / steps], [w / steps]], device=g.device).expand(2, B).contiguous()
        d = coef * g
        if every_step:
            return (None, None, None, *([d] * S))
        d_nll_only = torch.stack([d[0], torch.zeros_like(d[0])])
        return (None, None, None, *([d_nll_only] * (S - 1)), d)


def decode_loss(step_losses, steps: int, cov_weight: float, every_step: bool) -> torch.Tensor:
    return _DecodeLoss.apply(steps, cov_weight, every_step, *step_losses)


def decoder_open(tape, proj_a, proj_i, enc_a, enc_i, params):
    return _DecoderOpen.apply(tape, proj_a, proj_i, enc_a, enc_i, *params)


def decoder_step(tape, token, sent, h, cell, cov, mask_u8, target=None):
    return _DecoderStep.apply(tape, token, sent, h, cell, cov, mask_u8, target)


class _HighwayLayer(torch.autograd.Function):

    @staticmethod
    def forward(ctx, x2d, w_gate, b_gate, w_trans, b_trans):
        H = x2d.shape[1]
        w = _stacked([w_gate, w_trans], (2 * H, H))
        pre = torch.addmm(_stacked([b_gate, b_trans], (2 * H,)), x2d, w.t())
        y = ops.highway_fwd(pre, x2d)
        ctx.save_for_backward(x2d, pre, w)
        return y

    @staticmethod
    def backward(ctx, dy):
        x2d, pre, w = ctx.saved_tensors
        H = x2d.shape[1]
        d_pre, dx = ops.highway_bwd(pre, x2d, dy)
        dx = torch.addmm(dx, d_pre, w)
        with _leaf(d_pre, x2d):
            dw = tall_tn(d_pre, x2d)
        with _leaf(d_pre):
            db = ops.col_sum(d_pre)
        return dx, dw[:H], db[:H], dw[H:], db[H:]


def highway_layer(x: torch.Tensor, gate: torch.nn.Linear, transform: torch.nn.Linear) -> torch.Tensor:
    shape = x.shape
    y = _HighwayLayer.apply(x.reshape(-1, shape[-1]).contiguous(), gate.weight, gate.bias, transform.weight, transform.bias)
    return y.view(shape)
```

### mmbidaf_b200/layers/attention.py

```python
from __future__ import annotations

import weakref

import torch
import torch.nn as nn
import torch.nn.functional as F

from .. import functional as Fn
from .. import ops

__all__ = ["BiDAFAttention", "masked_softmax", "MultimodalAttentionDecoder"]


def _lib_fields():
    from .._lib import DECODER_WEIGHT_FIELDS
    return DECODER_WEIGHT_FIELDS


def _lin(attr, part):
    return lambda m: getattr(getattr(m, attr), part)


_FIELD_TO_PARAM = {}
for _f, _attr in (("W2", "W2"), ("Wc1", "Wc1"), ("v1", "v1"), ("W4", "W4"), ("Wc2", "Wc2"), ("v2", "v2")):
# ... 135 lines not shown
    def _param_of(self, field):
        return _FIELD_TO_PARAM[field](self)

    def forward(self, sent_embed, decoder_hidden, decoder_cell_state, text_audio_enc_out, text_img_enc_out,
                coverage_vec, mask):
        return self.step(sent_embed, decoder_hidden, decoder_cell_state, text_audio_enc_out, text_img_enc_out,
                         coverage_vec, mask)[:5]

    def greedy(self, emb_text, h0, enc_a, enc_i, mask, steps, target=None, text_len=None, no_repeat=False, min_sentences=0):
        if not enc_a.is_cuda:
            raise RuntimeError("mmbidaf_b200.layers.MultimodalAttentionDecoder runs on a B200 only (no CPU fallback)")
        if self.num_layers != 1:
            raise RuntimeError("MultimodalAttentionDecoder: only num_layers=1 is supported (the reference model uses 1)")
        constrained = bool(no_repeat) or min_sentences != 0
        if constrained and (target is not None or text_len is None):
            raise ValueError("greedy: a constrained roll-out needs text_len and takes no target (the eval loss is the unconstrained "
                             "roll-out's)")
        with torch.no_grad():
            seq = self._sequence(enc_a, enc_i)["seq"]
            B, Lt = seq.B, seq.Lt
            emb = emb_text.contiguous()
            h = h0.reshape(B, -1).contiguous()
            mask_u8 = ops._u8(mask)
            if constrained:
                probs, picks = ops.decoder_greedy_constrained_fwd(seq, emb, h, mask_u8, text_len.to(torch.int32).contiguous(), steps,
                                                                  no_repeat, min_sentences)
                return probs, picks, None
            tgt = None if target is None else target.reshape(B, -1).to(torch.int64).contiguous()
            if ops.decoder_cut(B, Lt) != "chunks":
                return ops.decoder_greedy_fwd(seq, emb, h, mask_u8, steps, tgt)
            if tgt is not None and tgt.shape[1] < steps:
                raise ValueError(f"greedy: {tgt.shape[1]} targets for {steps} steps")
            rows = torch.arange(B, device=h.device)
            sent = emb.new_zeros(B, emb.shape[2])
            cell = h.new_zeros(B, seq.H)
            cov = h.new_zeros(B, Lt)
            probs, picks, terms = [], [], []
            for s in range(steps):
                p, h, cell, _, cov, am, _, lossvec = ops.decoder_step_fwd(
                    seq, sent, h, cell, cov, mask_u8, want_argmax=True, target=None if tgt is None else tgt[:, s].contiguous())
                sent = emb[rows, am]
                probs.append(p)
                picks.append(am)
                terms.append(lossvec)
            return torch.stack(probs, 1), torch.stack(picks, 1), (torch.stack(terms) if tgt is not None else None)

    def beam(self, emb_text, h0, enc_a, enc_i, mask, text_len, steps, width, no_repeat=False, min_sentences=0):
        if not enc_a.is_cuda:
            raise RuntimeError("mmbidaf_b200.layers.MultimodalAttentionDecoder runs on a B200 only (no CPU fallback)")
        if self.num_layers != 1:
            raise RuntimeError("MultimodalAttentionDecoder: only num_layers=1 is supported (the reference model uses 1)")
        with torch.no_grad():
            seq = self._sequence(enc_a, enc_i)["seq"]
            B = seq.B
            return ops.decoder_beam_fwd(seq, emb_text.contiguous(), h0.reshape(B, -1).contiguous(), ops._u8(mask),
                                        text_len.to(torch.int32).contiguous(), steps, width, no_repeat, min_sentences)

    def beam_sample(self, emb_text, h0, enc_a, enc_i, mask, text_len, steps, width, key, temperature=1.0, no_repeat=False,
                    min_sentences=0):
        if not enc_a.is_cuda:
            raise RuntimeError("mmbidaf_b200.layers.MultimodalAttentionDecoder runs on a B200 only (no CPU fallback)")
        if self.num_layers != 1:
            raise RuntimeError("MultimodalAttentionDecoder: only num_layers=1 is supported (the reference model uses 1)")
        with torch.no_grad():
            seq = self._sequence(enc_a, enc_i)["seq"]
            B = seq.B
            return ops.decoder_beam_sample_fwd(seq, emb_text.contiguous(), h0.reshape(B, -1).contiguous(), ops._u8(mask),
                                               text_len.to(torch.int32).contiguous(), steps, width, key, temperature, no_repeat,
                                               min_sentences)

    def sample(self, emb_text, h0, enc_a, enc_i, mask, text_len, steps, num_samples, key, temperature=1.0, top_k=0, no_repeat=False,
               min_sentences=0, *, top_p=1.0):
        if not enc_a.is_cuda:
            raise RuntimeError("mmbidaf_b200.layers.MultimodalAttentionDecoder runs on a B200 only (no CPU fallback)")
        if self.num_layers != 1:
            raise RuntimeError("MultimodalAttentionDecoder: only num_layers=1 is supported (the reference model uses 1)")
        with torch.no_grad():
            seq = self._sequence(enc_a, enc_i)["seq"]
            B = seq.B
            return ops.decoder_sample_fwd(seq, emb_text.contiguous(), h0.reshape(B, -1).contiguous(), ops._u8(mask),
                                          text_len.to(torch.int32).contiguous(), steps, num_samples, key, temperature, top_k,
                                          no_repeat, min_sentences, top_p)

    def step(self, sent_embed, decoder_hidden, decoder_cell_state, text_audio_enc_out, text_img_enc_out, coverage_vec,
             mask, target=None):
        if not text_audio_enc_out.is_cuda:
            raise RuntimeError("mmbidaf_b200.layers.MultimodalAttentionDecoder runs on a B200 only (no CPU fallback)")
        if self.num_layers != 1:
            raise RuntimeError("MultimodalAttentionDecoder: only num_layers=1 is supported (the reference model uses 1)")
        seq = self._sequence(text_audio_enc_out, text_img_enc_out)
        B, Lt, _ = text_audio_enc_out.shape
        sent = sent_embed.reshape(B, -1).contiguous()
        h = decoder_hidden.reshape(B, -1).contiguous()
        cell = decoder_cell_state.reshape(B, -1).contiguous()
        cov = coverage_vec.reshape(B, Lt).contiguous()
        tgt = None if target is None else target.reshape(B).to(torch.int64).contiguous()
        if seq["tape"] is not None:
            prev = seq["last_h"]
            chained = prev is not None and (h is prev or h._base is prev)
            probs, h, cell, att, cov, lossvec = Fn.decoder_step(seq["tape"], None if chained else seq["token"], sent, h, cell,
                                                                cov, ops._u8(mask), tgt)
            seq["last_h"] = h
        else:
            probs, h, cell, att, cov, _, _, lossvec = ops.decoder_step_fwd(seq["seq"], sent, h, cell, cov, ops._u8(mask),
                                                                           target=tgt)
        return probs, h.unsqueeze(1), cell.unsqueeze(0), att.unsqueeze(2), cov.unsqueeze(2), (lossvec if tgt is not None else None)
```

### mmbidaf_b200/models.py

```python
from __future__ import annotations

import os

import torch
import torch.nn as nn

from . import functional as Fn
from . import ops
from .layers import BiDAFAttention, Embedding, ImageEmbedding, MultimodalAttentionDecoder, RNNEncoder

__all__ = ["MMBiDAF"]


class MMBiDAF(nn.Module):

    def __init__(self, hidden_size, text_embedding_size, audio_embedding_size, image_embedding_size, device,
                 drop_prob=0., max_transcript_length=405):
        super().__init__()
        self.device = device
        self.max_transcript_length = max_transcript_length
        self.emb = Embedding(embedding_size=text_embedding_size, hidden_size=hidden_size, drop_prob=drop_prob)
        self.a_emb = Embedding(embedding_size=audio_embedding_size, hidden_size=hidden_size, drop_prob=drop_prob)
        self.i_emb = Embedding(embedding_size=image_embedding_size, hidden_size=hidden_size, drop_prob=drop_prob)
        self.text_enc = RNNEncoder(input_size=hidden_size, hidden_size=hidden_size, num_layers=1, drop_prob=drop_prob)
        self.audio_enc = RNNEncoder(input_size=hidden_size, hidden_size=hidden_size, num_layers=1, drop_prob=drop_prob)
        self.image_enc = RNNEncoder(input_size=hidden_size, hidden_size=hidden_size, num_layers=1, drop_prob=drop_prob)
        self.image_keyframes_emb = ImageEmbedding()
        self.bidaf_att_audio = BiDAFAttention(2 * hidden_size, drop_prob=drop_prob)
        self.bidaf_att_image = BiDAFAttention(2 * hidden_size, drop_prob=drop_prob)
        self.mod_t_a = RNNEncoder(input_size=8 * hidden_size, hidden_size=hidden_size, num_layers=2, drop_prob=drop_prob)
        self.mod_t_i = RNNEncoder(input_size=8 * hidden_size, hidden_size=hidden_size, num_layers=2, drop_prob=drop_prob)
        self.multimodal_att_decoder = MultimodalAttentionDecoder(text_embedding_size, hidden_size,
                                                                 max_transcript_length, num_layers=1)

    use_streams = True
    stagger_encoders = os.environ.get("MMB_NO_STAGGER", "0") != "1"

    def _fork_join(self, jobs, meanwhile=None):
        if not (self.use_streams and torch.cuda.is_available()):
            results = [job() for job in jobs]
            if meanwhile is not None:
                meanwhile()
            return results
        main = torch.cuda.current_stream()
        if getattr(self, "_streams", None) is None or self._streams[0].device != main.device:
            object.__setattr__(self, "_streams", [torch.cuda.Stream(device=main.device, priority=-1 if i == 0 else 0)
                                                  for i in range(3)])
        results = []
        for stream, job in zip(self._streams, jobs):
            stream.wait_stream(main)
            with torch.cuda.stream(stream):
                results.append(job())
        if meanwhile is not None:
            meanwhile()
        capturing = torch.cuda.is_current_stream_capturing()
        for stream, res in zip(self._streams, results):
            main.wait_stream(stream)
            if capturing:
                continue
            for t in res:
                if isinstance(t, torch.Tensor):
                    t.record_stream(main)
        return results

    def load_state_dict(self, state_dict, strict=True, **kw):
        if state_dict and all(k.startswith("module.") for k in state_dict):
            state_dict = {k[len("module."):]: v for k, v in state_dict.items()}
        return super().load_state_dict(state_dict, strict=strict, **kw)

    def get_mask(self, X, X_len):
        from .layers.encoding import length_plan
        return length_plan(X_len, X.device).mask(X.size(1))[0]

    def forward(self, embedded_text, original_text_lengths, embedded_audio, original_audio_lengths, transformed_images,
                original_image_lengths, batch_target_indices, original_target_len, max_dec_len):
        B, Lt = embedded_text.size(0), embedded_text.size(1)
        steps = batch_target_indices.size(1) if self.training else max_dec_len
        start = {}

        def decoder_start():
            start["cell"] = embedded_text.new_zeros(1, B, self.mod_t_a.rnn.hidden_size)
            start["input"] = embedded_text.new_zeros(B, 1, embedded_text.size(-1))
            start["cov"] = embedded_text.new_zeros(B, Lt, 1)
            start["rows"] = torch.arange(B, device=embedded_text.device)
            start["targets"] = batch_target_indices.reshape(B, -1).to(embedded_text.device).long()
            start["targets_t"] = start["targets"].t().contiguous()
            if self.training:
                start["next"] = embedded_text[start["rows"].unsqueeze(0), start["targets"][:, :steps].t()]
            self.multimodal_att_decoder.prepare()

        mod_text_audio, mod_text_image, decoder_hidden, decoder_mask = self._encode(
            embedded_text, original_text_lengths, embedded_audio, original_audio_lengths, transformed_images, original_image_lengths,
            decoder_start)
        decoder_cell_state, decoder_input, coverage_vec = start["cell"], start["input"], start["cov"]
        rows, targets, targets_t = start["rows"], start["targets"], start["targets_t"]
        out_distributions, step_losses = [], []
        if self.training:
            next_inputs = start["next"]
        for idx in range(steps):
            tgt = targets_t[idx] if idx < targets_t.size(0) else targets[:, idx]
            out_distribution, decoder_hidden, decoder_cell_state, att_cov_dist, coverage_vec, step_loss = \
                self.multimodal_att_decoder.step(decoder_input, decoder_hidden, decoder_cell_state, mod_text_audio,
                                                 mod_text_image, coverage_vec, decoder_mask, target=tgt)
            if self.training:
                decoder_input = next_inputs[idx].unsqueeze(1)
            else:
                decoder_input = embedded_text[rows, out_distribution.max(dim=1)[1]].unsqueeze(1)
            out_distributions.append(out_distribution)
            step_losses.append(step_loss)
        cov_loss_wt = 1.0
        loss = Fn.decode_loss(step_losses, steps, cov_loss_wt, self.training)
        return torch.stack(out_distributions).transpose(0, 1), loss

    def summarize(self, text, text_len, audio, audio_len, images, image_len, max_dec_len, targets=None, beam_width=None,
                  no_repeat=False, min_sentences=0, num_samples=None, temperature=1.0, top_k=0, seed=None, top_p=1.0, replacement=True):
        from .layers.encoding import length_plan
        from .summarize import Beams, Inclusion, Samples, Summary, best_sample, check_options, sample_logp
        check_options("summarize", targets is not None, beam_width, no_repeat, min_sentences, num_samples, temperature, top_k, seed,
                      top_p, replacement)
        constrained = no_repeat or min_sentences > 0
        was_training = self.training
        self.eval()
        try:
            with torch.no_grad():
                B = text.size(0)
                dec = self.multimodal_att_decoder
                start = {}

                def decoder_start():
                    if targets is not None:
                        start["targets"] = targets.reshape(B, -1).to(text.device).long()
                    dec.prepare()

                enc_a, enc_i, h0, mask = self._encode(text, text_len, audio, audio_len, images, image_len, decoder_start)
                if num_samples is not None:
                    lens = length_plan(text_len, text.device).len_i32
                    key = ops.rng_next_keys(text.device, 1) if seed is None else ops.seed_key(seed, text.device)
                    if not replacement:
                        _, _, scores, rows, phi, keys, paths, slots, kappa = dec.beam_sample(
                            text, h0, enc_a, enc_i, mask, lens, max_dec_len, num_samples, key, temperature, no_repeat, min_sentences)
                        M = rows.shape[-1]
                        idx = slots.long().clamp_min(0).unsqueeze(3).expand(-1, -1, -1, M)
                        probs = rows.transpose(1, 2).gather(1, idx) * (slots >= 0).unsqueeze(3)
                        samples = Samples(paths, probs, scores[:, -1])
                        sel, cnt = ops.greedy_select(paths.view(B * num_samples, -1), lens.repeat_interleave(num_samples))
                        best_probs, indices, counts = best_sample(samples, sel, cnt)
                        return Summary(best_probs, None, indices, counts, None, samples, Inclusion(phi[:, -1], keys[:, -1], kappa))
                    probs, tokens = dec.sample(text, h0, enc_a, enc_i, mask, lens, max_dec_len, num_samples, key, temperature, top_k,
                                               no_repeat, min_sentences, top_p=top_p)
                    samples = Samples(tokens, probs, sample_logp(probs, tokens, lens))
                    sel, cnt = ops.greedy_select(tokens.view(B * num_samples, -1), lens.repeat_interleave(num_samples))
                    best_probs, indices, counts = best_sample(samples, sel, cnt)
                    return Summary(best_probs, None, indices, counts, None, samples)
                if beam_width is not None:
                    lens = length_plan(text_len, text.device).len_i32
                    tokens, parents, scores, rows, best, path = dec.beam(text, h0, enc_a, enc_i, mask, lens, max_dec_len, beam_width,
                                                                         no_repeat, min_sentences)
                    M = rows.shape[-1]
                    probs = rows.gather(2, path.long().clamp_min(0)[:, :, None, None].expand(-1, -1, 1, M)).squeeze(2)
                    indices, counts = ops.greedy_select(best, lens)
                    return Summary(probs, None, indices, counts, Beams(tokens, parents, scores, rows))
                if constrained:
                    lens = length_plan(text_len, text.device).len_i32
                    probs, picks, _ = dec.greedy(text, h0, enc_a, enc_i, mask, max_dec_len, text_len=lens, no_repeat=no_repeat,
                                                 min_sentences=min_sentences)
                    indices, counts = ops.greedy_select(picks, lens)
                    return Summary(probs, None, indices, counts)
                probs, argmax, terms = dec.greedy(text, h0, enc_a, enc_i, mask, max_dec_len, target=start.get("targets"))
                loss = None if terms is None else Fn.decode_loss(list(terms.unbind(0)), max_dec_len, 1.0, False)
                indices, counts = ops.greedy_select(argmax, length_plan(text_len, text.device).len_i32)
        finally:
            self.train(was_training)
        return Summary(probs, loss, indices, counts)

    def _encode(self, embedded_text, original_text_lengths, embedded_audio, original_audio_lengths, transformed_images,
                original_image_lengths, decoder_start):
        B, Lt = embedded_text.size(0), embedded_text.size(1)

        def text_branch():
            emb = self.emb(embedded_text)
            return emb, self.text_enc(emb, original_text_lengths)[0]

        def audio_branch():
            return (self.audio_enc(self.a_emb(embedded_audio), original_audio_lengths)[0],)

        def image_branch():
            img = transformed_images.reshape(-1, *transformed_images.shape[2:])
            feats = self.image_keyframes_emb(img).reshape(B, transformed_images.size(1), -1)
            return feats, self.image_enc(self.i_emb(feats), original_image_lengths)[0]

        masks = {}

        def make_masks():
# ... 100 lines not shown
```

### mmbidaf_b200/ops.py

```python
from __future__ import annotations

import contextlib
import ctypes
import math
import os
from typing import Optional, Tuple

import torch

from . import _lib

PREC_FP32, PREC_BF16 = 0, 1
launch_count = 0


def _count(n: int) -> None:
    global launch_count
    launch_count += n


def _u8(mask: Optional[torch.Tensor]) -> Optional[torch.Tensor]:
    if mask is None:
        return None
    if mask.dtype == torch.bool:
# ... 193 lines not shown
        self.Wh_stack = torch.cat([P["lstm_w_hh"], self.Wh4], dim=0).contiguous()
        self.bcat = (P["lstm_b_ih"] + P["lstm_b_hh"]).contiguous()
        self.out_w, self.out_b = P["out_w"].contiguous(), P["out_b"].contiguous()
        self.Wh4t, self.Wcatt, self.out_wt = self.Wh4.t().contiguous(), self.Wcat.t().contiguous(), self.out_w.t().contiguous()
        self.Wb13t = self.Wb13.transpose(1, 2).contiguous()
        self.Mp = (self.M + 7) // 8 * 8
        self.out_w_pad = torch.cat([self.out_w, self.out_w.new_zeros(self.Mp - self.M, self.H)], dim=0).contiguous()
        flat = lambda k: P[k].reshape(-1).contiguous()
        self.v1, self.wc1, self.v2, self.wc2 = flat("v1"), flat("Wc1"), flat("v2"), flat("Wc2")
        self.vb1, self.vb2 = flat("vb1"), flat("vb2")
        self.v1b, self.v2b, self.vb1b, self.vb2b = flat("v1b"), flat("v2b"), flat("vb1b"), flat("vb2b")


class DecoderSeq:

    def __init__(self, params: dict, enc_a, enc_i, proj_a, proj_i, out_size: int, weights: Optional[DecoderWeights] = None):
        w = weights if weights is not None else DecoderWeights(params, out_size)
        self.__dict__.update(w.__dict__)
        self.enc_a, self.enc_i = enc_a.detach().contiguous(), enc_i.detach().contiguous()
        self.proj_a, self.proj_i = proj_a.detach().contiguous(), proj_i.detach().contiguous()
        self.B, self.Lt, D = self.enc_a.shape
        if D != self.D or out_size != self.M:
            raise RuntimeError(f"DecoderSeq: encoder width {D} / output size {out_size} do not match the weights ({self.D}, {self.M})")
        self.nch = _lib.lib().mmb_decoder_chunks(self.B, self.Lt)
        self.counters = torch.zeros(2, self.B, device=self.enc_a.device, dtype=torch.int32)


def decoder_cut(B: int, Lt: int) -> str:
    cut = os.environ.get("MMB_DECODER_CUT")
    if cut is None:
        cut = "fused" if B * Lt <= 20000 else "chunks"
    return cut


def decoder_step_fwd(seq: DecoderSeq, sent, h, cell, coverage, mask_u8, want_argmax: bool = False, target=None):
    lib = _lib.lib()
    B, Lt, D, H, E, M, nch = seq.B, seq.Lt, seq.D, seq.H, seq.E, seq.M, seq.nch
    f32 = dict(device=h.device, dtype=torch.float32)
    p = _lib.ptr
    st = _lib.stream()
    cut = decoder_cut(B, Lt)
    if cut != "chunks":
        hw, alpha, beta = torch.empty(B, 4 * D, **f32), torch.empty(B, 2, Lt, **f32), torch.empty(B, 2, **f32)
        ctx12, pb = torch.empty(2, B, D, **f32), torch.empty(2, B, D, **f32)
        xcat, gates = torch.empty(B, D + E + H, **f32), torch.empty(B, 4 * H, **f32)
        probs, h_out, cell_out = torch.empty(B, M, **f32), torch.empty(B, H, **f32), torch.empty(B, H, **f32)
        att_cov, cov_out = torch.empty(B, Lt, **f32), torch.empty(B, Lt, **f32)
        argmax = torch.empty(B, device=h.device, dtype=torch.int64) if want_argmax else None
        lossvec = torch.empty(2, B, **f32) if target is not None else None
        _lib.check(lib.mmb_decoder_step_fused_fwd(
            p(seq.proj_a), p(seq.proj_i), p(seq.enc_a), p(seq.enc_i), p(seq.Wh4t), p(seq.bh4), p(seq.v1), p(seq.wc1), p(seq.v2),
            p(seq.wc2), p(seq.v1b), p(seq.v2b), p(seq.Wb13t), p(seq.vb1), p(seq.vb2), p(seq.vb1b), p(seq.vb2b), p(seq.Wcatt),
            p(seq.bcat), p(seq.out_wt), p(seq.out_b), p(sent), p(h), p(cell), p(coverage), p(mask_u8), p(target), p(probs), p(h_out),
            p(cell_out), p(att_cov), p(cov_out), p(argmax), p(None if lossvec is None else lossvec[0]),
            p(None if lossvec is None else lossvec[1]), p(hw), p(alpha), p(beta), p(ctx12), p(pb), p(xcat), p(gates),
            B, Lt, D, H, E, M, st), "mmb_decoder_step_fused_fwd")
        _count(1)
        return probs, h_out, cell_out, att_cov, cov_out, argmax, (hw, alpha, beta, ctx12, pb, xcat, gates), lossvec
    hw = torch.addmm(seq.bh4, h, seq.Wh4.t())
    alpha = torch.empty(B, 2, Lt, **f32)
    stats, ctxp = torch.empty(B, nch, 4, **f32), torch.empty(B, nch, 2, D, **f32)
    ctx12, scale = torch.empty(2, B, D, **f32), torch.empty(B, 2, nch, **f32)
    _lib.check(lib.mmb_decoder_attn_fwd(p(seq.proj_a), p(seq.proj_i), p(seq.enc_a), p(seq.enc_i), p(hw), p(coverage),
                                        p(seq.v1), p(seq.wc1), p(seq.v2), p(seq.wc2), p(seq.v1b), p(seq.v2b), p(alpha),
                                        p(stats), p(ctxp), p(ctx12), p(scale), p(seq.counters[0]), B, Lt, D, nch, st),
               "mmb_decoder_attn_fwd")
    pb = torch.bmm(ctx12, seq.Wb13.transpose(1, 2))
    xcat = torch.empty(B, D + E + H, **f32)
    att_cov, cov_out, beta = torch.empty(B, Lt, **f32), torch.empty(B, Lt, **f32), torch.empty(B, 2, **f32)
    lossvec = torch.empty(2, B, **f32) if target is not None else None
    _lib.check(lib.mmb_decoder_attn_finish(p(pb), p(hw), p(ctx12), p(scale), p(coverage), p(sent), p(h), p(seq.vb1),
                                           p(seq.vb2), p(seq.vb1b), p(seq.vb2b), p(alpha), p(xcat), p(att_cov),
                                           p(cov_out), p(beta), p(None if lossvec is None else lossvec[1]),
                                           B, Lt, D, E, H, nch, st), "mmb_decoder_attn_finish")
    gates = torch.addmm(seq.bcat, xcat, seq.Wcat.t())
    h_out, cell_out = torch.empty(B, H, **f32), torch.empty(B, H, **f32)
    _lib.check(lib.mmb_decoder_cell_fwd(p(gates), p(cell), p(h_out), p(cell_out), B, H, st), "mmb_decoder_cell_fwd")
    probs = torch.addmm(seq.out_b, h_out, seq.out_w.t())
    argmax = torch.empty(B, device=h.device, dtype=torch.int64) if want_argmax else None
    _lib.check(lib.mmb_decoder_out_softmax(p(probs), p(mask_u8), p(argmax), p(target),
                                           p(None if lossvec is None else lossvec[0]), B, M, st), "mmb_decoder_out_softmax")
    _count(5)
    return probs, h_out, cell_out, att_cov, cov_out, argmax, (hw, alpha, beta, ctx12, pb, xcat, gates), lossvec


def decoder_greedy_fwd(seq: DecoderSeq, emb_text, h0, mask_u8, steps: int, target=None):
    lib = _lib.lib()
    B, Lt, D, H, E, M = seq.B, seq.Lt, seq.D, seq.H, seq.E, seq.M
    dev = h0.device
    if emb_text.shape != (B, Lt, E) or h0.shape != (B, H) or mask_u8.shape != (B, M):
        raise ValueError(f"decoder_greedy_fwd: emb_text {tuple(emb_text.shape)}, h0 {tuple(h0.shape)}, mask {tuple(mask_u8.shape)} "
                         f"for B={B} Lt={Lt} E={E} H={H} M={M}")
    T = 0
    if target is not None:
        T = target.shape[1]
        if target.dtype != torch.int64 or target.shape[0] != B or T < steps:
            raise ValueError(f"decoder_greedy_fwd: target {tuple(target.shape)} {target.dtype} for B={B}, {steps} steps")
    probs = torch.empty(B, steps, M, device=dev, dtype=torch.float32)
    argmax = torch.empty(B, steps, device=dev, dtype=torch.int64)
    terms = torch.empty(steps, 2, B, device=dev, dtype=torch.float32) if target is not None else None
    p = _lib.ptr
    _lib.check(lib.mmb_decoder_greedy_fused(
        p(seq.proj_a), p(seq.proj_i), p(seq.enc_a), p(seq.enc_i), p(seq.Wh4t), p(seq.bh4), p(seq.v1), p(seq.wc1), p(seq.v2),
        p(seq.wc2), p(seq.v1b), p(seq.v2b), p(seq.Wb13t), p(seq.vb1), p(seq.vb2), p(seq.vb1b), p(seq.vb2b), p(seq.Wcatt),
        p(seq.bcat), p(seq.out_wt), p(seq.out_b), p(emb_text), p(h0), p(mask_u8), p(target), p(probs), p(argmax), p(terms),
        B, Lt, D, H, E, M, int(steps), int(T), _lib.stream()), "mmb_decoder_greedy_fused")
    _count(1)
    return probs, argmax, terms


def _check_constraints(who: str, no_repeat, min_sentences) -> None:
    if not isinstance(no_repeat, int) or no_repeat not in (0, 1):
        raise ValueError(f"{who}: no_repeat {no_repeat!r}, expected a bool")
    if isinstance(min_sentences, bool) or not isinstance(min_sentences, int) or min_sentences < 0:
        raise ValueError(f"{who}: min_sentences {min_sentences!r}, expected an int >= 0")


def decoder_greedy_constrained_fwd(seq: DecoderSeq, emb_text, h0, mask_u8, text_len_i32, steps: int, no_repeat: bool = False,
                                   min_sentences: int = 0):
    lib = _lib.lib()
    B, Lt, D, H, E, M = seq.B, seq.Lt, seq.D, seq.H, seq.E, seq.M
    dev = h0.device
    _check_constraints("decoder_greedy_constrained_fwd", no_repeat, min_sentences)
    if int(steps) <= 0:
        raise ValueError(f"decoder_greedy_constrained_fwd: {steps} steps")
    if emb_text.shape != (B, Lt, E) or h0.shape != (B, H) or mask_u8.shape != (B, M) or text_len_i32.shape != (B,):
        raise ValueError(f"decoder_greedy_constrained_fwd: emb_text {tuple(emb_text.shape)}, h0 {tuple(h0.shape)}, "
                         f"mask {tuple(mask_u8.shape)}, text_len {tuple(text_len_i32.shape)} for B={B} Lt={Lt} E={E} H={H} M={M}")
    if text_len_i32.dtype != torch.int32:
        raise ValueError(f"decoder_greedy_constrained_fwd: text_len {text_len_i32.dtype}, not int32")
    S = int(steps)
    probs = torch.empty(B, S, M, device=dev, dtype=torch.float32)
    picks = torch.empty(B, S, device=dev, dtype=torch.int64)
    p = _lib.ptr
    _lib.check(lib.mmb_decoder_greedy_constrained_fused(
        p(seq.proj_a), p(seq.proj_i), p(seq.enc_a), p(seq.enc_i), p(seq.Wh4t), p(seq.bh4), p(seq.v1), p(seq.wc1), p(seq.v2),
        p(seq.wc2), p(seq.v1b), p(seq.v2b), p(seq.Wb13t), p(seq.vb1), p(seq.vb2), p(seq.vb1b), p(seq.vb2b), p(seq.Wcatt),
        p(seq.bcat), p(seq.out_wt), p(seq.out_b), p(emb_text), p(h0), p(mask_u8), p(text_len_i32), p(probs), p(picks),
        B, Lt, D, H, E, M, S, int(no_repeat), int(min_sentences), _lib.stream()), "mmb_decoder_greedy_constrained_fused")
    _count(1)
    return probs, picks


BEAM_MAX_WIDTH = 8


def decoder_beam_fwd(seq: DecoderSeq, emb_text, h0, mask_u8, text_len_i32, steps: int, width: int, no_repeat: bool = False,
                     min_sentences: int = 0, constrained: Optional[bool] = None):
    lib = _lib.lib()
    B, Lt, D, H, E, M = seq.B, seq.Lt, seq.D, seq.H, seq.E, seq.M
    dev = h0.device
    if not 1 <= int(width) <= BEAM_MAX_WIDTH:
        raise ValueError(f"decoder_beam_fwd: beam width {width} (1..{BEAM_MAX_WIDTH})")
    if int(steps) <= 0:
        raise ValueError(f"decoder_beam_fwd: {steps} steps")
    _check_constraints("decoder_beam_fwd", no_repeat, min_sentences)
    if emb_text.shape != (B, Lt, E) or h0.shape != (B, H) or mask_u8.shape != (B, M) or text_len_i32.shape != (B,):
        raise ValueError(f"decoder_beam_fwd: emb_text {tuple(emb_text.shape)}, h0 {tuple(h0.shape)}, mask {tuple(mask_u8.shape)}, "
                         f"text_len {tuple(text_len_i32.shape)} for B={B} Lt={Lt} E={E} H={H} M={M}")
    if text_len_i32.dtype != torch.int32:
        raise ValueError(f"decoder_beam_fwd: text_len {text_len_i32.dtype}, not int32")
    S, K = int(steps), int(width)
    tokens = torch.empty(B, S, K, device=dev, dtype=torch.int64)
    parents = torch.empty(B, S, K, device=dev, dtype=torch.int32)
    scores = torch.empty(B, S, K, device=dev, dtype=torch.float32)
    probs = torch.empty(B, S, K, M, device=dev, dtype=torch.float32)
# ... 302 lines not shown
```

Measured before the change: 7533.

## Batch teacher-forced decoder output head across all steps, separating recurrent step kernels

Adds a teacher-forced training path in which each decoder step kernel runs only the recurrent attention and LSTM cell, skipping the per-step output projection and softmax. The vocabulary projection, softmax and NLL for all T steps are then computed in one batched head kernel that processes several rows per block and reuses each weight load across them. The backward pass is restructured the same way, with one batched head backward producing dh for every step before the per-step recurrent backward kernels. This removes the per-step output-head matvec from the sequential critical path, at the cost of new kernels, extra buffers and a separate code path used only during training.

```diff
diff --git a/include/mmbidaf_b200.h b/include/mmbidaf_b200.h
--- a/include/mmbidaf_b200.h
+++ b/include/mmbidaf_b200.h
@@ -188,6 +188,31 @@
                                        const float* v2, const float* wc2, float* d_proj_a, float* d_proj_i, float* d_cov,
                                        const float* Wh_stack, float* d_h, int B, int Lt, int D, int H, int M, mmb_stream_t stream);
 
+MMB_API int mmb_decoder_teacher_step_fwd(const float* proj_a, const float* proj_i, const float* enc_a, const float* enc_i,
+                                         const float* Wh4t, const float* bh4, const float* v1, const float* wc1, const float* v2,
+                                         const float* wc2, const float* v1b, const float* v2b, const float* Wb13t, const float* vb1,
+                                         const float* vb2, const float* vb1b, const float* vb2b, const float* Wcatt,
+                                         const float* bcat, const float* sent, const float* h, const float* cell, const float* cov,
+                                         float* h_out, float* cell_out, float* att_cov, float* cov_out, float* cov_loss, float* hw,
+                                         float* alpha, float* beta, float* ctx12, float* pb, float* xcat, float* gates, int B, int Lt,
+                                         int D, int H, int E, int M, mmb_stream_t stream);
+MMB_API int mmb_decoder_teacher_head_fwd(const float* h_out, const float* out_wt, const float* out_b, const uint8_t* mask,
+                                         const long long* target, float* probs, float* nll, int ldn, int T, int B, int H, int M,
+                                         mmb_stream_t stream);
+MMB_API int mmb_decoder_teacher_head_bwd(const float* probs, const float* d_probs, const long long* target, const float* g_nll,
+                                         int ldn, const float* out_w, float* d_logits, int ldd, float* dh_head, int T, int B, int Lt,
+                                         int D, int H, int M, mmb_stream_t stream);
+MMB_API int mmb_decoder_teacher_step_bwd(const float* dh_head, const float* g_cov, const float* gates, const float* cell_in,
+                                         const float* cell_out, const float* d_h_out, const float* d_cell_out, const float* Wcat_ctx,
+                                         const float* d_cov_out, const float* alpha, const float* beta, const float* ctx12,
+                                         const float* pb, const float* hw, const float* vb1, const float* vb2, const float* att,
+                                         const float* cov_out, const float* Wb13, float* d_gates, int ldg, float* d_cell, float* datt,
+                                         float* dcov_tot, float* d_pre_b, float* d_ctx12, float* vec_acc, float* scal_acc,
+                                         const float* proj_a, const float* proj_i, const float* enc_a, const float* enc_i,
+                                         const float* coverage, const float* v1, const float* wc1, const float* v2, const float* wc2,
+                                         float* d_proj_a, float* d_proj_i, float* d_cov, const float* Wh_stack, float* d_h, int B,
+                                         int Lt, int D, int H, int M, mmb_stream_t stream);
+
 MMB_API int mmb_decoder_attn_bwd(const float* proj_a, const float* proj_i, const float* enc_a, const float* enc_i,
                                  const float* hw, const float* coverage, const float* alpha, const float* beta,
                                  const float* datt, const float* d_ctx12, const float* d_cov_out, const float* d_pre_b,
diff --git a/mmbidaf_b200/_lib.py b/mmbidaf_b200/_lib.py
--- a/mmbidaf_b200/_lib.py
+++ b/mmbidaf_b200/_lib.py
@@ -50,6 +50,10 @@
     "mmb_decoder_cell_bwd": [c_void_p] * 7 + [c_int] + [c_void_p] + [c_int] * 2 + [c_void_p],
     "mmb_decoder_attn_finish_bwd": [c_void_p, c_int] + [c_void_p] * 18 + [c_int] * 3 + [c_void_p],
     "mmb_decoder_step_fused_bwd": [c_void_p] * 25 + [c_int] + [c_void_p] + [c_int] + [c_void_p] * 21 + [c_int] * 5 + [c_void_p],
+    "mmb_decoder_teacher_step_fwd": [c_void_p] * 35 + [c_int] * 6 + [c_void_p],
+    "mmb_decoder_teacher_head_fwd": [c_void_p] * 7 + [c_int] * 5 + [c_void_p],
+    "mmb_decoder_teacher_head_bwd": [c_void_p] * 4 + [c_int] + [c_void_p] * 2 + [c_int] + [c_void_p] + [c_int] * 6 + [c_void_p],
+    "mmb_decoder_teacher_step_bwd": [c_void_p] * 20 + [c_int] + [c_void_p] * 21 + [c_int] * 5 + [c_void_p],
     "mmb_decoder_attn_bwd": [c_void_p] * 24 + [c_int] + [c_void_p] * 3 + [c_int] * 4 + [c_void_p],
     "mmb_highway_fwd": [c_void_p] * 3 + [ctypes.c_longlong, c_int, c_void_p],
     "mmb_highway_bwd": [c_void_p] * 5 + [ctypes.c_longlong, c_int, c_void_p],
diff --git a/mmbidaf_b200/csrc/decoder_fused.cu b/mmbidaf_b200/csrc/decoder_fused.cu
--- a/mmbidaf_b200/csrc/decoder_fused.cu
+++ b/mmbidaf_b200/csrc/decoder_fused.cu
@@ -358,7 +358,8 @@
   return cut;
 }
 
-template <bool kGreedy, bool kBeam = false, bool kConstrained = false, bool kSample = false, bool kNucleus = false, bool kStoch = false>
+template <bool kGreedy, bool kBeam = false, bool kConstrained = false, bool kSample = false, bool kNucleus = false, bool kStoch = false,
+          bool kTeacher = false>
 __device__ __forceinline__ void dec_fused_body(const FusedArgs& a, const GreedyArgs& g, const BeamArgs& bm, const ConstraintArgs& cn,
                                                const SampleArgs sp, const NucleusArgs nu = NucleusArgs{}, const StochArgs st = StochArgs{}) {
   cg::cluster_group cluster = cg::this_cluster();
@@ -796,7 +797,8 @@
         float* gs = a.gates + (size_t)b * 4 * H;
         gs[j] = gi; gs[H + j] = gf; gs[2 * H + j] = gg; gs[3 * H + j] = go;
       }
-      for (int r = 0; r < CL; ++r) cluster.map_shared_rank(s_hn, r)[j] = hn;
+      if constexpr (!kTeacher)
+        for (int r = 0; r < CL; ++r) cluster.map_shared_rank(s_hn, r)[j] = hn;
     }
   }
   DEC_STAMP(12);
@@ -812,7 +814,7 @@
     a.cov_loss[lrow] = cs;
   }
 
-  {
+  if constexpr (!kTeacher) {
     const int per = (M + CL - 1) / CL, m0 = min(M, R * per), m1 = min(M, m0 + per);
     float* const lg = s_cpart;
     block_matvec_t(a.out_wt, M, a.out_b, s_hn, H, m1 - m0, s_scr, SCR, (m0 & 3) == 0, [&](int i) { return m0 + i; }, [&](int i, float v) { lg[i] = v; });
@@ -1252,6 +1254,10 @@
   dec_fused_body<false>(a, GreedyArgs{}, BeamArgs{}, ConstraintArgs{}, SampleArgs{});
 }
 
+__global__ void __launch_bounds__(NT) dec_teacher_step_kernel(const FusedArgs a) {
+  dec_fused_body<false, false, false, false, false, false, true>(a, GreedyArgs{}, BeamArgs{}, ConstraintArgs{}, SampleArgs{});
+}
+
 __global__ void __launch_bounds__(NT) dec_greedy_fused_kernel(const FusedArgs a, const GreedyArgs g) {
   dec_fused_body<true>(a, g, BeamArgs{}, ConstraintArgs{}, SampleArgs{});
 }
@@ -1328,7 +1334,8 @@
   int stage_off;
 };
 
-__global__ void __launch_bounds__(NT) dec_bwd_head_kernel(const HeadArgs a) {
+template <bool kTeacher>
+__device__ __forceinline__ void dec_bwd_body(const HeadArgs& a) {
   cg::cluster_group cluster = cg::this_cluster();
   const int CL = (int)cluster.num_blocks(), R = (int)cluster.block_rank();
   const int b = blockIdx.x / CL;
@@ -1367,6 +1374,7 @@
     }
   }
   DEC_STAMP(18);
+  if constexpr (!kTeacher) {
   const int m0 = min(M, R * per_m), m1 = min(M, m0 + per_m);
   const int tg = a.target ? (int)a.target[b] : -1;
   const float dp_t = a.target ? -a.g_nll[b] / (a.probs[(size_t)b * M + tg] + 1e-12f) : 0.f;
@@ -1399,11 +1407,14 @@
   if (m1 - m0 <= 0 && tid < H)
     for (int r = 0; r < CL; ++r) cluster.map_shared_rank(s_dhp, r)[R * H + tid] = 0.f;
   cluster.sync();
+  }
   DEC_STAMP(20);
   if (tid < H) {
     const int j = tid;
     float dh = 0.f;
-    for (int r = 0; r < CL; ++r) dh += s_dhp[r * H + j];
+    if constexpr (kTeacher) dh = a.probs[(size_t)b * H + j];
+    else
+      for (int r = 0; r < CL; ++r) dh += s_dhp[r * H + j];
     if (a.d_h_out) dh += a.d_h_out[(size_t)b * H + j];
     const float* g = a.gates + (size_t)b * 4 * H;
     const float gi = g[j], gf = g[H + j], gg = g[2 * H + j], go = g[3 * H + j];
@@ -1768,6 +1779,192 @@
   DEC_STAMP(27);
 }
 
+__global__ void __launch_bounds__(NT) dec_bwd_head_kernel(const HeadArgs a) { dec_bwd_body<false>(a); }
+
+__global__ void __launch_bounds__(NT) dec_bwd_teacher_kernel(const HeadArgs a) { dec_bwd_body<true>(a); }
+
+constexpr int kHeadRows = 4;
+
+static size_t teacher_head_smem(int H, int M, bool bwd) {
+  return ((size_t)kHeadRows * (bwd ? M : H) + (bwd ? 0 : (size_t)kHeadRows * M) + 32) * sizeof(float);
+}
+
+__device__ __forceinline__ void matvec_like_block(const float* __restrict__ W, size_t ldw, const float* x, int ldx, int K, int n_out,
+                                                  int scratch_cap, bool quads, float* y) {
+  float v[kHeadRows];
+#pragma unroll
+  for (int r = 0; r < kHeadRows; ++r) v[r] = 0.f;
+  if (quads) {
+    const int S = max(1, min(min(NT / (n_out >> 2), scratch_cap / n_out), K));
+    const int per = (K + S - 1) / S;
+    for (int sl = 0; sl < S; ++sl) {
+      const int k0 = min(K, sl * per), k1 = min(K, k0 + per);
+      float acc[kHeadRows];
+#pragma unroll
+      for (int r = 0; r < kHeadRows; ++r) acc[r] = 0.f;
+      for (int k = k0; k < k1; ++k) {
+        const float w = __ldg(W + (size_t)k * ldw);
+#pragma unroll
+        for (int r = 0; r < kHeadRows; ++r) acc[r] = fmaf(w, x[r * ldx + k], acc[r]);
+      }
+#pragma unroll
+      for (int r = 0; r < kHeadRows; ++r) v[r] += acc[r];
+    }
+  } else {
+    const int S = max(1, min(min(NT / n_out, scratch_cap / n_out), 32));
+    const int per = (K + S - 1) / S;
+    for (int sl = 0; sl < S; ++sl) {
+      const int k0 = min(K, sl * per), k1 = min(K, k0 + per);
+      float a0[kHeadRows], a1[kHeadRows], a2[kHeadRows], a3[kHeadRows];
+#pragma unroll
+      for (int r = 0; r < kHeadRows; ++r) a0[r] = a1[r] = a2[r] = a3[r] = 0.f;
+      const int len = k1 - k0, n4 = len / 16 * 4 + (len % 16 >= 8 ? 2 : 0);
+      int k = k0;
+      for (int g = 0; g < n4; ++g, k += 4) {
+        float w[4];
+#pragma unroll
+        for (int u = 0; u < 4; ++u) w[u] = __ldg(W + (size_t)(k + u) * ldw);
+#pragma unroll
+        for (int r = 0; r < kHeadRows; ++r) {
+          a0[r] = fmaf(w[0], x[r * ldx + k], a0[r]); a1[r] = fmaf(w[1], x[r * ldx + k + 1], a1[r]);
+          a2[r] = fmaf(w[2], x[r * ldx + k + 2], a2[r]); a3[r] = fmaf(w[3], x[r * ldx + k + 3], a3[r]);
+        }
+      }
+      for (; k < k1; ++k) {
+        const float w = __ldg(W + (size_t)k * ldw);
+#pragma unroll
+        for (int r = 0; r < kHeadRows; ++r) a0[r] = fmaf(w, x[r * ldx + k], a0[r]);
+      }
+#pragma unroll
+      for (int r = 0; r < kHeadRows; ++r) {
+        const float acc = (a0[r] + a1[r]) + (a2[r] + a3[r]);
+        v[r] = sl == 0 ? acc : v[r] + acc;
+      }
+    }
+  }
+#pragma unroll
+  for (int r = 0; r < kHeadRows; ++r) y[r] = v[r];
+}
+
+__global__ void __launch_bounds__(NT) dec_teacher_head_kernel(const float* __restrict__ h_out, const float* __restrict__ out_wt,
+                                                              const float* __restrict__ out_b, const uint8_t* __restrict__ mask,
+                                                              const long long* __restrict__ target, float* __restrict__ probs,
+                                                              float* __restrict__ nll, int ldn, int T, int B, int H, int M, int CL) {
+  extern __shared__ __align__(16) float smem[];
+  float* s_h = smem;
+  float* s_lg = s_h + kHeadRows * H;
+  float* s_red = s_lg + kHeadRows * M;
+  const int tid = threadIdx.x;
+  const int r0 = blockIdx.x * kHeadRows, nr = min(kHeadRows, T * B - r0);
+  for (int i = tid; i < kHeadRows * H; i += NT) s_h[i] = i < nr * H ? h_out[(size_t)r0 * H + i] : 0.f;
+  __syncthreads();
+  const int per = (M + CL - 1) / CL;
+  for (int m = tid; m < M; m += NT) {
+    const int m0 = m / per * per, n_out = min(M, m0 + per) - m0;
+    const bool quads = (m0 & 3) == 0 && ((M | n_out) & 3) == 0 && (reinterpret_cast<uintptr_t>(out_wt) & 15) == 0 && SCR >= 2 * n_out;
+    float y[kHeadRows];
+    matvec_like_block(out_wt + m, M, s_h, H, H, n_out, SCR, quads, y);
+    const float bias = __ldg(out_b + m);
+#pragma unroll
+    for (int r = 0; r < kHeadRows; ++r)
+      if (r < nr) s_lg[r * M + m] = mask[(size_t)((r0 + r) % B) * M + m] ? y[r] + bias : kNegFill;
+  }
+  __syncthreads();
+  for (int r = 0; r < nr; ++r) {
+    const int row = r0 + r, t = row / B, b = row - t * B;
+    const float* lg = s_lg + r * M;
+    float gmx = -INFINITY, gsum = 0.f, mx[MAXC], sm[MAXC];
+    for (int q = 0; q < CL; ++q) {
+      const int m0 = min(M, q * per), m1 = min(M, m0 + per);
+      float v = -INFINITY;
+      for (int m = m0 + tid; m < m1; m += NT) v = fmaxf(v, lg[m]);
+      mx[q] = block_max(v, s_red);
+      float su = 0.f;
+      for (int m = m0 + tid; m < m1; m += NT) su += expf(lg[m] - mx[q]);
+      sm[q] = block_sum(su, s_red);
+      if (m0 < M) gmx = fmaxf(gmx, mx[q]);
+    }
+    for (int q = 0; q < CL; ++q)
+      if (min(M, q * per) < M) gsum = fmaf(sm[q], expf(mx[q] - gmx), gsum);
+    const float inv = 1.f / gsum;
+    const int tg = target ? (int)target[row] : -1;
+    float* prow = probs + ((size_t)b * T + t) * M;
+    for (int m = tid; m < M; m += NT) {
+      const float p = expf(lg[m] - gmx) * inv;
+      prow[m] = p;
+      if (m == tg) nll[(size_t)t * ldn + b] = -logf(p + 1e-12f);
+    }
+  }
+}
+
+__global__ void __launch_bounds__(NT) dec_teacher_head_bwd_kernel(const float* __restrict__ probs, const float* __restrict__ d_probs,
+                                                                  const long long* __restrict__ target, const float* __restrict__ g_nll,
+                                                                  int ldn, const float* __restrict__ out_w, float* __restrict__ d_logits,
+                                                                  int ldd, float* __restrict__ dh_head, int T, int B, int H, int M, int CL,
+                                                                  int mv_cap) {
+  extern __shared__ __align__(16) float smem[];
+  float* s_dl = smem;
+  float* s_red = s_dl + kHeadRows * M;
+  const int tid = threadIdx.x;
+  const int r0 = blockIdx.x * kHeadRows, nr = min(kHeadRows, T * B - r0);
+  const int per = (M + CL - 1) / CL;
+  for (int r = 0; r < kHeadRows; ++r) {
+    if (r >= nr) {
+      for (int m = tid; m < M; m += NT) s_dl[r * M + m] = 0.f;
+      continue;
+    }
+    const int row = r0 + r, t = row / B, b = row - t * B;
+    const float* p = probs + ((size_t)b * T + t) * M;
+    const float* dp = d_probs ? d_probs + ((size_t)b * T + t) * M : nullptr;
+    const int tg = target ? (int)target[row] : -1;
+    const float dp_t = target ? -g_nll[(size_t)t * ldn + b] / (p[tg] + 1e-12f) : 0.f;
+    float dot = 0.f;
+    if (dp)
+      for (int q = 0; q < CL; ++q) {
+        const int m0 = min(M, q * per), m1 = min(M, m0 + per);
+        float v = 0.f;
+        for (int m = m0 + tid; m < m1; m += NT) v = fmaf(p[m], dp[m], v);
+        dot += block_sum(v, s_red);
+      }
+    if (target) dot = fmaf(p[tg], dp_t, dot);
+    for (int m = tid; m < M; m += NT) {
+      const float d = (dp ? dp[m] : 0.f) + (m == tg ? dp_t : 0.f);
+      const float v = p[m] * (d - dot);
+      s_dl[r * M + m] = v;
+      d_logits[(size_t)row * ldd + m] = v;
+    }
+    for (int m = M + tid; m < ldd; m += NT) d_logits[(size_t)row * ldd + m] = 0.f;
+  }
+  __syncthreads();
+  for (int j = tid; j < H; j += NT) {
+    float dh[kHeadRows];
+#pragma unroll
+    for (int r = 0; r < kHeadRows; ++r) dh[r] = 0.f;
+    for (int q = 0; q < CL; ++q) {
+      const int m0 = min(M, q * per), K = min(M, m0 + per) - m0;
+      const bool quads = (H & 3) == 0 && (reinterpret_cast<uintptr_t>(out_w + (size_t)m0 * H) & 15) == 0 && mv_cap >= 2 * H;
+      float y[kHeadRows];
+      matvec_like_block(out_w + (size_t)m0 * H + j, H, s_dl + m0, M, K, H, mv_cap, quads, y);
+#pragma unroll
+      for (int r = 0; r < kHeadRows; ++r) dh[r] += K > 0 ? y[r] + 0.f : 0.f;
+    }
+    for (int r = 0; r < nr; ++r) dh_head[(size_t)(r0 + r) * H + j] = dh[r];
+  }
+}
+
+static int launch_teacher_head(bool bwd, const void* fn, void** args, int T, int B, int H, int M, mmb_stream_t stream, const char* who) {
+  static size_t smem_set[2] = {0, 0};
+  const size_t smem = teacher_head_smem(H, M, bwd);
+  MMB_REQUIRE(smem <= 200 * 1024, MMB_ERR_UNSUPPORTED, "%s: %zu B of shared memory (M=%d)", who, smem, M);
+  if (smem > 48 * 1024 && smem > smem_set[bwd]) {
+    MMB_CUDA(cudaFuncSetAttribute(fn, cudaFuncAttributeMaxDynamicSharedMemorySize, (int)smem));
+    smem_set[bwd] = smem;
+  }
+  const unsigned grid = (unsigned)((T * B + kHeadRows - 1) / kHeadRows);
+  MMB_CUDA(cudaLaunchKernel(fn, dim3(grid), dim3(NT), args, smem, static_cast<cudaStream_t>(stream)));
+  return check_launch(who);
+}
+
 static size_t g_head_smem_set = 0;
 
 static size_t head_smem_bytes(int D, int H, int M, int CL, int chunk = 0, bool sweeps = false, int PW = NW) {
@@ -1812,7 +2009,7 @@
 
 static int launch_fused(FusedArgs a, const GreedyArgs* g, const char* who, mmb_stream_t stream, BeamArgs* bm = nullptr,
                         const ConstraintArgs* cn = nullptr, SampleArgs* sp = nullptr, NucleusArgs* nu = nullptr,
-                        StochArgs* sb = nullptr) {
+                        StochArgs* sb = nullptr, bool teacher = false) {
   const int B = a.B, Lt = a.Lt, D = a.D, H = a.H, E = a.E, M = a.M;
   MMB_REQUIRE(B > 0 && Lt > 0 && D > 0 && H > 0 && E >= 0 && M > 0, MMB_ERR_INVALID,
               "%s: B=%d Lt=%d D=%d H=%d E=%d M=%d", who, B, Lt, D, H, E, M);
@@ -1853,10 +2050,10 @@
       smem = (base_floats + stage_floats) * 4;
     }
   }
-  static size_t smem_set[11] = {0, 0, 0, 0, 0, 0, 0, 0, 0, 0, 0};
-  const int which = sb ? (cn ? 10 : 9) : nu ? (cn ? 8 : 7) : sp ? (cn ? 6 : 5) : bm ? (cn ? 4 : 2) : g ? (cn ? 3 : 1) : 0;
+  static size_t smem_set[12] = {0, 0, 0, 0, 0, 0, 0, 0, 0, 0, 0, 0};
+  const int which = teacher ? 11 : sb ? (cn ? 10 : 9) : nu ? (cn ? 8 : 7) : sp ? (cn ? 6 : 5) : bm ? (cn ? 4 : 2) : g ? (cn ? 3 : 1) : 0;
   if (smem > smem_set[which]) {
-    const void* fn = which == 10 ? (const void*)dec_beam_sample_constrained_kernel : which == 9 ? (const void*)dec_beam_sample_kernel
+    const void* fn = which == 11 ? (const void*)dec_teacher_step_kernel : which == 10 ? (const void*)dec_beam_sample_constrained_kernel : which == 9 ? (const void*)dec_beam_sample_kernel
                    : which == 8 ? (const void*)dec_sample_nucleus_constrained_kernel : which == 7 ? (const void*)dec_sample_nucleus_kernel
                    : which == 6 ? (const void*)dec_sample_constrained_kernel : which == 5 ? (const void*)dec_sample_kernel
                    : which == 4 ? (const void*)dec_beam_constrained_kernel : which == 3 ? (const void*)dec_greedy_constrained_kernel
@@ -1884,6 +2081,10 @@
   attr[0].val.clusterDim.z = 1;
   cfg.attrs = attr;
   cfg.numAttrs = 1;
+  if (teacher) {
+    MMB_CUDA(cudaLaunchKernelEx(&cfg, dec_teacher_step_kernel, a));
+    return check_launch("dec_teacher_step_kernel");
+  }
   if (sb && cn) {
     MMB_CUDA(cudaLaunchKernelEx(&cfg, dec_beam_sample_constrained_kernel, a, *g, *bm, *cn, *sb));
     return check_launch("dec_beam_sample_constrained_kernel");
@@ -2181,6 +2382,59 @@
   return check_launch("dec_bwd_head_kernel");
 }
 
+namespace mmb {
+static bool bwd_row_stage(int B, int Lt, int D, int H, int M, bool aligned, size_t* base_floats, size_t* stage_floats) {
+  static const char* stage_env = getenv("MMB_DEC_STAGE");
+  const int CL = (long long)B * 4 * 2 <= 160 ? 8 : 4;
+  const int chunk = (Lt + CL - 1) / CL;
+  *base_floats = (head_smem_bytes(D, H, M, CL, chunk, true, NW / 2) - 64) / 4;
+  *stage_floats = 4 + 2 * (((size_t)chunk * D + 3) & ~(size_t)3);
+  return (D & 3) == 0 && aligned && (*base_floats + *stage_floats) * 4 + 64 <= 227 * 1024 && !(stage_env && atoi(stage_env) == 0);
+}
+
+static int launch_step_bwd(HeadArgs a, bool teacher, const char* who, mmb_stream_t stream) {
+  const int B = a.B, D = a.D, H = a.H, M = a.M, Lt = a.Lt, chunk = a.chunk;
+  const int CL = (long long)B * 4 * 2 <= 160 ? 8 : 4;
+  size_t smem = head_smem_bytes(D, H, M, CL, chunk, true);
+  MMB_REQUIRE(smem <= 200 * 1024, MMB_ERR_UNSUPPORTED, "%s: %zu B of shared memory (Lt=%d)", who, smem, Lt);
+  {
+    const bool aligned = ((reinterpret_cast<uintptr_t>(a.proj_a) | reinterpret_cast<uintptr_t>(a.proj_i) | reinterpret_cast<uintptr_t>(a.enc_a) |
+                           reinterpret_cast<uintptr_t>(a.enc_i) | reinterpret_cast<uintptr_t>(a.d_proj_a) |
+                           reinterpret_cast<uintptr_t>(a.d_proj_i)) & 15) == 0;
+    size_t base_floats = 0, stage_floats = 0;
+    if (bwd_row_stage(B, Lt, D, H, M, aligned, &base_floats, &stage_floats)) {
+      a.stage_off = (int)base_floats;
+      smem = (base_floats + stage_floats) * 4 + 64;
+    }
+  }
+  static size_t g_teacher_smem_set = 0;
+  size_t& smem_set = teacher ? g_teacher_smem_set : g_head_smem_set;
+  if (smem > smem_set) {
+    MMB_CUDA(cudaFuncSetAttribute(teacher ? dec_bwd_teacher_kernel : dec_bwd_head_kernel, cudaFuncAttributeMaxDynamicSharedMemorySize,
+                                  (int)smem));
+    smem_set = smem;
+  }
+  cudaLaunchConfig_t cfg{};
+  cfg.gridDim = dim3((unsigned)(B * CL));
+  cfg.blockDim = dim3(NT);
+  cfg.dynamicSmemBytes = smem;
+  cfg.stream = static_cast<cudaStream_t>(stream);
+  cudaLaunchAttribute attr[1];
+  attr[0].id = cudaLaunchAttributeClusterDimension;
+  attr[0].val.clusterDim.x = (unsigned)CL;
+  attr[0].val.clusterDim.y = 1;
+  attr[0].val.clusterDim.z = 1;
+  cfg.attrs = attr;
+  cfg.numAttrs = 1;
+  if (teacher) {
+    MMB_CUDA(cudaLaunchKernelEx(&cfg, dec_bwd_teacher_kernel, a));
+    return check_launch("dec_bwd_teacher_kernel");
+  }
+  MMB_CUDA(cudaLaunchKernelEx(&cfg, dec_bwd_head_kernel, a));
+  return check_launch("dec_bwd_head_kernel (whole step)");
+}
+}
+
 extern "C" int mmb_decoder_step_fused_bwd(const float* probs, const float* d_probs, const long long* target, const float* g_nll,
                                           const float* g_cov, const float* out_w, const float* gates, const float* cell_in,
                                           const float* cell_out, const float* d_h_out, const float* d_cell_out, const float* Wcat_ctx,
@@ -2206,36 +2460,77 @@
              alpha, beta, ctx12, pb, hw, vb1, vb2, att, cov_out, Wb13, d_logits, d_gates, d_cell, datt, dcov_tot, d_pre_b, d_ctx12,
              vec_acc, scal_acc, B, Lt, D, H, M, ldd, ldg, chunk,
              1, proj_a, proj_i, enc_a, enc_i, coverage, v1, wc1, v2, wc2, d_proj_a, d_proj_i, d_cov, Wh_stack, d_h, 0};
-  size_t smem = head_smem_bytes(D, H, M, CL, chunk, true);
-  MMB_REQUIRE(smem <= 200 * 1024, MMB_ERR_UNSUPPORTED, "mmb_decoder_step_fused_bwd: %zu B of shared memory (Lt=%d)", smem, Lt);
-  {
-    static const char* stage_env = getenv("MMB_DEC_STAGE");
-    const size_t base_floats = (head_smem_bytes(D, H, M, CL, chunk, true, NW / 2) - 64) / 4;
-    const size_t stage_floats = 4 + 2 * (((size_t)chunk * D + 3) & ~(size_t)3);
-    const bool aligned = ((reinterpret_cast<uintptr_t>(proj_a) | reinterpret_cast<uintptr_t>(proj_i) | reinterpret_cast<uintptr_t>(enc_a) |
-                           reinterpret_cast<uintptr_t>(enc_i) | reinterpret_cast<uintptr_t>(d_proj_a) |
-                           reinterpret_cast<uintptr_t>(d_proj_i)) & 15) == 0;
-    if ((D & 3) == 0 && aligned && (base_floats + stage_floats) * 4 + 64 <= 227 * 1024 && !(stage_env && atoi(stage_env) == 0)) {
-      a.stage_off = (int)base_floats;
-      smem = (base_floats + stage_floats) * 4 + 64;
-    }
-  }
-  if (smem > g_head_smem_set) {
-    MMB_CUDA(cudaFuncSetAttribute(dec_bwd_head_kernel, cudaFuncAttributeMaxDynamicSharedMemorySize, (int)smem));
-    g_head_smem_set = smem;
-  }
-  cudaLaunchConfig_t cfg{};
-  cfg.gridDim = dim3((unsigned)(B * CL));
-  cfg.blockDim = dim3(NT);
-  cfg.dynamicSmemBytes = smem;
-  cfg.stream = static_cast<cudaStream_t>(stream);
-  cudaLaunchAttribute attr[1];
-  attr[0].id = cudaLaunchAttributeClusterDimension;
-  attr[0].val.clusterDim.x = (unsigned)CL;
-  attr[0].val.clusterDim.y = 1;
-  attr[0].val.clusterDim.z = 1;
-  cfg.attrs = attr;
-  cfg.numAttrs = 1;
-  MMB_CUDA(cudaLaunchKernelEx(&cfg, dec_bwd_head_kernel, a));
-  return check_launch("dec_bwd_head_kernel (whole step)");
-}
+  return launch_step_bwd(a, false, "mmb_decoder_step_fused_bwd", stream);
+}
+
+extern "C" int mmb_decoder_teacher_step_fwd(const float* proj_a, const float* proj_i, const float* enc_a, const float* enc_i,
+                                            const float* Wh4t, const float* bh4, const float* v1, const float* wc1, const float* v2,
+                                            const float* wc2, const float* v1b, const float* v2b, const float* Wb13t, const float* vb1,
+                                            const float* vb2, const float* vb1b, const float* vb2b, const float* Wcatt,
+                                            const float* bcat, const float* sent, const float* h, const float* cell, const float* cov, float* h_out,
+                                            float* cell_out, float* att_cov, float* cov_out, float* cov_loss, float* hw, float* alpha,
+                                            float* beta, float* ctx12, float* pb, float* xcat, float* gates, int B, int Lt, int D, int H,
+                                            int E, int M, mmb_stream_t stream) {
+  using namespace mmb;
+  MMB_REQUIRE(proj_a && proj_i && enc_a && enc_i && Wh4t && bh4 && v1 && wc1 && v2 && wc2 && v1b && v2b && Wb13t && vb1 && vb2 &&
+                  vb1b && vb2b && Wcatt && bcat && sent && h && cell && cov && h_out && cell_out && att_cov && cov_out && cov_loss && hw &&
+                  alpha && beta && ctx12 && pb && xcat && gates,
+              MMB_ERR_INVALID, "mmb_decoder_teacher_step_fwd: null pointer");
+  FusedArgs a{proj_a, proj_i, enc_a, enc_i, Wh4t, bh4, v1, wc1, v2, wc2, v1b, v2b, Wb13t, vb1, vb2, vb1b, vb2b, Wcatt, bcat, nullptr,
+              nullptr, sent, h, cell, cov, nullptr, nullptr, nullptr, h_out, cell_out, att_cov, cov_out, nullptr, nullptr, cov_loss, hw,
+              alpha, beta, ctx12, pb, xcat, gates, B, Lt, D, H, E, M, 0, 0};
+  return launch_fused(a, nullptr, "mmb_decoder_teacher_step_fwd", stream, nullptr, nullptr, nullptr, nullptr, nullptr, true);
+}
+
+extern "C" int mmb_decoder_teacher_head_fwd(const float* h_out, const float* out_wt, const float* out_b, const uint8_t* mask,
+                                            const long long* target, float* probs, float* nll, int ldn, int T, int B, int H, int M,
+                                            mmb_stream_t stream) {
+  using namespace mmb;
+  MMB_REQUIRE(h_out && out_wt && out_b && mask && probs && (!target || nll), MMB_ERR_INVALID, "mmb_decoder_teacher_head_fwd: null pointer");
+  MMB_REQUIRE(T > 0 && B > 0 && H > 0 && M > 0 && (!target || ldn >= B), MMB_ERR_INVALID,
+              "mmb_decoder_teacher_head_fwd: T=%d B=%d H=%d M=%d ldn=%d", T, B, H, M, ldn);
+  int CL = (long long)B * 4 * 2 <= 160 ? 8 : 4;
+  void* args[] = {&h_out, &out_wt, &out_b, &mask, &target, &probs, &nll, &ldn, &T, &B, &H, &M, &CL};
+  return launch_teacher_head(false, (const void*)dec_teacher_head_kernel, args, T, B, H, M, stream, "dec_teacher_head_kernel");
+}
+
+extern "C" int mmb_decoder_teacher_head_bwd(const float* probs, const float* d_probs, const long long* target, const float* g_nll,
+                                            int ldn, const float* out_w, float* d_logits, int ldd, float* dh_head, int T, int B, int Lt,
+                                            int D, int H, int M, mmb_stream_t stream) {
+  using namespace mmb;
+  MMB_REQUIRE(probs && out_w && d_logits && dh_head && (!target || g_nll), MMB_ERR_INVALID, "mmb_decoder_teacher_head_bwd: null pointer");
+  MMB_REQUIRE(T > 0 && B > 0 && Lt > 0 && D > 0 && H > 0 && H <= NT && M > 0 && ldd >= M && (!target || ldn >= B), MMB_ERR_INVALID,
+              "mmb_decoder_teacher_head_bwd: T=%d B=%d Lt=%d D=%d H=%d M=%d ldd=%d ldn=%d", T, B, Lt, D, H, M, ldd, ldn);
+  int CL = (long long)B * 4 * 2 <= 160 ? 8 : 4;
+  size_t base_floats = 0, stage_floats = 0;
+  int mv_cap = (bwd_row_stage(B, Lt, D, H, M, true, &base_floats, &stage_floats) ? NW / 2 : NW) * 3 * D;
+  void* args[] = {&probs, &d_probs, &target, &g_nll, &ldn, &out_w, &d_logits, &ldd, &dh_head, &T, &B, &H, &M, &CL, &mv_cap};
+  return launch_teacher_head(true, (const void*)dec_teacher_head_bwd_kernel, args, T, B, H, M, stream, "dec_teacher_head_bwd_kernel");
+}
+
+extern "C" int mmb_decoder_teacher_step_bwd(const float* dh_head, const float* g_cov, const float* gates, const float* cell_in,
+                                            const float* cell_out, const float* d_h_out, const float* d_cell_out, const float* Wcat_ctx,
+                                            const float* d_cov_out, const float* alpha, const float* beta, const float* ctx12,
+                                            const float* pb, const float* hw, const float* vb1, const float* vb2, const float* att,
+                                            const float* cov_out, const float* Wb13, float* d_gates, int ldg, float* d_cell, float* datt,
+                                            float* dcov_tot, float* d_pre_b, float* d_ctx12, float* vec_acc, float* scal_acc,
+                                            const float* proj_a, const float* proj_i, const float* enc_a, const float* enc_i,
+                                            const float* coverage, const float* v1, const float* wc1, const float* v2, const float* wc2,
+                                            float* d_proj_a, float* d_proj_i, float* d_cov, const float* Wh_stack, float* d_h, int B,
+                                            int Lt, int D, int H, int M, mmb_stream_t stream) {
+  using namespace mmb;
+  MMB_REQUIRE(dh_head && gates && cell_in && cell_out && Wcat_ctx && alpha && beta && ctx12 && pb && hw && vb1 && vb2 && Wb13 &&
+                  d_gates && d_cell && datt && dcov_tot && d_pre_b && d_ctx12 && vec_acc && scal_acc && proj_a && proj_i && enc_a &&
+                  enc_i && coverage && v1 && wc1 && v2 && wc2 && d_proj_a && d_proj_i && d_cov && Wh_stack && d_h,
+              MMB_ERR_INVALID, "mmb_decoder_teacher_step_bwd: null pointer");
+  MMB_REQUIRE(!g_cov || (att && cov_out), MMB_ERR_INVALID, "mmb_decoder_teacher_step_bwd: loss-term pointers");
+  MMB_REQUIRE(B > 0 && Lt > 0 && D > 0 && D <= 256 && H > 0 && M > 0 && ldg >= 4 * H + 4 * D && H <= NT, MMB_ERR_INVALID,
+              "mmb_decoder_teacher_step_bwd: B=%d Lt=%d D=%d H=%d M=%d ldg=%d", B, Lt, D, H, M, ldg);
+  const int CL = (long long)B * 4 * 2 <= 160 ? 8 : 4;
+  const int chunk = (Lt + CL - 1) / CL;
+  HeadArgs a{dh_head, nullptr, nullptr, nullptr, g_cov, nullptr, gates, cell_in, cell_out, d_h_out, d_cell_out, Wcat_ctx, nullptr,
+             d_cov_out, alpha, beta, ctx12, pb, hw, vb1, vb2, att, cov_out, Wb13, nullptr, d_gates, d_cell, datt, dcov_tot, d_pre_b,
+             d_ctx12, vec_acc, scal_acc, B, Lt, D, H, M, 0, ldg, chunk,
+             1, proj_a, proj_i, enc_a, enc_i, coverage, v1, wc1, v2, wc2, d_proj_a, d_proj_i, d_cov, Wh_stack, d_h, 0};
+  return launch_step_bwd(a, true, "mmb_decoder_teacher_step_bwd", stream);
+}
diff --git a/mmbidaf_b200/functional.py b/mmbidaf_b200/functional.py
--- a/mmbidaf_b200/functional.py
+++ b/mmbidaf_b200/functional.py
@@ -393,6 +393,50 @@
         return None, (tape.zero_token(d_h) if ctx.has_token else None), None, d_h, d_cell, d_cov, None, None
 
 
+class _DecoderTeacher(torch.autograd.Function):
+
+    @staticmethod
+    def forward(ctx, tape, token, h0, cell0, cov0, sent0, next_inputs, mask_u8, targets_t):
+        probs, terms, hs, cells, covs, att, saved = ops.decoder_teacher_fwd(tape.seq, sent0, next_inputs, h0, cell0, cov0, mask_u8,
+                                                                            targets_t)
+        ctx.tape = tape
+        ctx.save_for_backward(h0, cell0, cov0, hs, cells, covs, att, probs, targets_t, *saved)
+        ctx.set_materialize_grads(False)
+        return probs, hs[-1], cells[-1], covs[-1], terms
+
+    @staticmethod
+    def backward(ctx, d_probs, d_h_out, d_cell_out, d_cov_out, d_terms):
+        tape = ctx.tape
+        if getattr(tape, "closed", False) or getattr(ctx, "consumed", False):
+            raise RuntimeError("mmbidaf_b200: the teacher-forced decoder's backward ran twice over one forward (retain_graph=True is not "
+                               "supported)")
+        ctx.consumed = True
+        h0, cell0, cov0, hs, cells, covs, att, probs, targets_t, *saved = ctx.saved_tensors
+        T = hs.shape[0]
+        d_terms = None if d_terms is None else d_terms.contiguous()
+        d_logits, dh_head = ops.decoder_teacher_head_bwd(tape.seq, probs, d_probs, None if d_terms is None else targets_t,
+                                                         None if d_terms is None else d_terms[:, 0])
+        tape.open_accumulators()
+        r = tape.rows
+        M = tape.seq.M
+        d_h, d_cell, d_cov = d_h_out, d_cell_out, d_cov_out
+        for t in range(T - 1, -1, -1):
+            h, cell, cov = (h0, cell0, cov0) if t == 0 else (hs[t - 1], cells[t - 1], covs[t - 1])
+            st = [x[t] for x in saved]
+            d_h, d_cell, d_cov, d_gates, d_ctx12, d_hw4, d_pre_b = ops.decoder_teacher_step_bwd(
+                tape.seq, h, cell, cov, cells[t], st, dh_head[t], d_h, d_cell, d_cov, tape.d_proj_a, tape.d_proj_i, tape.vec_acc,
+                tape.scal_acc, g_cov=None if d_terms is None else d_terms[t, 1], att_cov=att[t], cov_out=covs[t])
+            hw, alpha, beta, ctx12, pb, xcat, gates = st
+            r["h_prev"].append(h); r["xcat"].append(xcat); r["h_out"].append(hs[t]); r["alpha"].append(alpha)
+            r["dlog"].append(d_logits[t, :, :M]); r["da"].append(d_gates); r["dctx12"].append(d_ctx12); r["dhw4"].append(d_hw4)
+            r["dpre"].append(d_pre_b); r["ctx12"].append(ctx12)
+        return None, tape.zero_token(d_h), d_h, d_cell, d_cov, None, None, None, None
+
+
+def decoder_teacher_forced(tape, token, h0, cell0, cov0, sent0, next_inputs, mask_u8, targets_t):
+    return _DecoderTeacher.apply(tape, token, h0, cell0, cov0, sent0, next_inputs, mask_u8, targets_t)
+
+
 class _DecodeLoss(torch.autograd.Function):
 
     _coef = {}
diff --git a/mmbidaf_b200/layers/attention.py b/mmbidaf_b200/layers/attention.py
--- a/mmbidaf_b200/layers/attention.py
+++ b/mmbidaf_b200/layers/attention.py
@@ -241,6 +241,20 @@
                                           text_len.to(torch.int32).contiguous(), steps, num_samples, key, temperature, top_k,
                                           no_repeat, min_sentences, top_p)
 
+    def teacher_forced(self, sent0, next_inputs, decoder_hidden, decoder_cell_state, text_audio_enc_out, text_img_enc_out,
+                       coverage_vec, mask, targets):
+        if not text_audio_enc_out.is_cuda:
+            raise RuntimeError("mmbidaf_b200.layers.MultimodalAttentionDecoder runs on a B200 only (no CPU fallback)")
+        seq = self._sequence(text_audio_enc_out, text_img_enc_out)
+        if seq["tape"] is None:
+            raise RuntimeError("teacher_forced: a training op -- it needs autograd on the encoder outputs (use step() or greedy())")
+        B, Lt, _ = text_audio_enc_out.shape
+        probs, h, cell, cov, terms = Fn.decoder_teacher_forced(
+            seq["tape"], seq["token"], decoder_hidden.reshape(B, -1).contiguous(), decoder_cell_state.reshape(B, -1).contiguous(),
+            coverage_vec.reshape(B, Lt).contiguous(), sent0.reshape(B, -1).contiguous(), next_inputs.contiguous(), ops._u8(mask),
+            targets.to(torch.int64).contiguous())
+        return probs, h.unsqueeze(1), cell.unsqueeze(0), cov.unsqueeze(2), terms
+
     def step(self, sent_embed, decoder_hidden, decoder_cell_state, text_audio_enc_out, text_img_enc_out, coverage_vec,
              mask, target=None):
         if not text_audio_enc_out.is_cuda:
diff --git a/mmbidaf_b200/models.py b/mmbidaf_b200/models.py
--- a/mmbidaf_b200/models.py
+++ b/mmbidaf_b200/models.py
@@ -77,6 +77,7 @@
         B, Lt = embedded_text.size(0), embedded_text.size(1)
         steps = batch_target_indices.size(1) if self.training else max_dec_len
         start = {}
+        teacher = self.training and torch.is_grad_enabled() and embedded_text.is_cuda and ops.decoder_cut(B, Lt) == "fused"
 
         def decoder_start():
             start["cell"] = embedded_text.new_zeros(1, B, self.mod_t_a.rnn.hidden_size)
@@ -94,6 +95,12 @@
             decoder_start)
         decoder_cell_state, decoder_input, coverage_vec = start["cell"], start["input"], start["cov"]
         rows, targets, targets_t = start["rows"], start["targets"], start["targets_t"]
+        cov_loss_wt = 1.0
+        if teacher:
+            out, _, _, _, terms = self.multimodal_att_decoder.teacher_forced(
+                decoder_input, start["next"], decoder_hidden, decoder_cell_state, mod_text_audio, mod_text_image, coverage_vec,
+                decoder_mask, targets_t[:steps])
+            return out, Fn.decode_loss(list(terms.unbind(0)), steps, cov_loss_wt, True)
         out_distributions, step_losses = [], []
         if self.training:
             next_inputs = start["next"]
@@ -108,7 +115,6 @@
                 decoder_input = embedded_text[rows, out_distribution.max(dim=1)[1]].unsqueeze(1)
             out_distributions.append(out_distribution)
             step_losses.append(step_loss)
-        cov_loss_wt = 1.0
         loss = Fn.decode_loss(step_losses, steps, cov_loss_wt, self.training)
         return torch.stack(out_distributions).transpose(0, 1), loss
 
diff --git a/mmbidaf_b200/ops.py b/mmbidaf_b200/ops.py
--- a/mmbidaf_b200/ops.py
+++ b/mmbidaf_b200/ops.py
@@ -299,6 +299,75 @@
                                            p(None if lossvec is None else lossvec[0]), B, M, st), "mmb_decoder_out_softmax")
     _count(5)
     return probs, h_out, cell_out, att_cov, cov_out, argmax, (hw, alpha, beta, ctx12, pb, xcat, gates), lossvec
+
+
+def decoder_teacher_fwd(seq: DecoderSeq, sent0, next_inputs, h0, cell0, cov0, mask_u8, targets_t):
+    lib = _lib.lib()
+    B, Lt, D, H, E, M = seq.B, seq.Lt, seq.D, seq.H, seq.E, seq.M
+    T = targets_t.shape[0]
+    if targets_t.shape != (T, B) or T < 1 or (T > 1 and next_inputs.shape[0] < T - 1):
+        raise ValueError(f"decoder_teacher_fwd: targets {tuple(targets_t.shape)}, next {tuple(next_inputs.shape)} for B={B}")
+    f32 = dict(device=h0.device, dtype=torch.float32)
+    p = _lib.ptr
+    st = _lib.stream()
+    hs, cells, covs, att = (torch.empty(T, B, H, **f32), torch.empty(T, B, H, **f32), torch.empty(T, B, Lt, **f32),
+                            torch.empty(T, B, Lt, **f32))
+    hw, alpha, beta = torch.empty(T, B, 4 * D, **f32), torch.empty(T, B, 2, Lt, **f32), torch.empty(T, B, 2, **f32)
+    ctx12, pb = torch.empty(T, 2, B, D, **f32), torch.empty(T, 2, B, D, **f32)
+    xcat, gates = torch.empty(T, B, D + E + H, **f32), torch.empty(T, B, 4 * H, **f32)
+    terms = torch.empty(T, 2, B, **f32)
+    for t in range(T):
+        h, cell, cov = (h0, cell0, cov0) if t == 0 else (hs[t - 1], cells[t - 1], covs[t - 1])
+        _lib.check(lib.mmb_decoder_teacher_step_fwd(
+            p(seq.proj_a), p(seq.proj_i), p(seq.enc_a), p(seq.enc_i), p(seq.Wh4t), p(seq.bh4), p(seq.v1), p(seq.wc1), p(seq.v2),
+            p(seq.wc2), p(seq.v1b), p(seq.v2b), p(seq.Wb13t), p(seq.vb1), p(seq.vb2), p(seq.vb1b), p(seq.vb2b), p(seq.Wcatt), p(seq.bcat),
+            p(sent0 if t == 0 else next_inputs[t - 1]), p(h), p(cell), p(cov), p(hs[t]), p(cells[t]), p(att[t]), p(covs[t]),
+            p(terms[t, 1]), p(hw[t]), p(alpha[t]), p(beta[t]), p(ctx12[t]), p(pb[t]), p(xcat[t]), p(gates[t]), B, Lt, D, H, E, M, st),
+            "mmb_decoder_teacher_step_fwd")
+    probs = torch.empty(B, T, M, **f32)
+    _lib.check(lib.mmb_decoder_teacher_head_fwd(p(hs), p(seq.out_wt), p(seq.out_b), p(mask_u8), p(targets_t), p(probs), p(terms),
+                                                2 * B, T, B, H, M, st), "mmb_decoder_teacher_head_fwd")
+    _count(T + 1)
+    return probs, terms, hs, cells, covs, att, (hw, alpha, beta, ctx12, pb, xcat, gates)
+
+
+def decoder_teacher_head_bwd(seq: DecoderSeq, probs, d_probs, targets_t, g_nll):
+    B, H, M = seq.B, seq.H, seq.M
+    T = probs.shape[1]
+    f32 = dict(device=probs.device, dtype=torch.float32)
+    d_logits, dh_head = torch.empty(T, B, seq.Mp, **f32), torch.empty(T, B, H, **f32)
+    p = _lib.ptr
+    ldn = g_nll.stride(0) if g_nll is not None else 0
+    if g_nll is not None and (not g_nll.is_cuda or g_nll.stride(1) != 1 or targets_t is None):
+        raise ValueError("decoder_teacher_head_bwd: g_nll needs targets and contiguous rows on the device")
+    _lib.check(_lib.lib().mmb_decoder_teacher_head_bwd(
+        p(probs), p(None if d_probs is None else d_probs.contiguous()), p(targets_t),
+        None if g_nll is None else g_nll.data_ptr(), ldn, p(seq.out_w), p(d_logits), seq.Mp,
+        p(dh_head), T, B, seq.Lt, seq.D, H, M, _lib.stream()), "mmb_decoder_teacher_head_bwd")
+    _count(1)
+    return d_logits, dh_head
+
+
+def decoder_teacher_step_bwd(seq: DecoderSeq, h, cell, coverage, cell_out, saved, dh_head, d_h_out, d_cell_out, d_cov_out,
+                             d_proj_a, d_proj_i, vec_acc, scal_acc, g_cov=None, att_cov=None, cov_out=None):
+    B, Lt, D, H, M = seq.B, seq.Lt, seq.D, seq.H, seq.M
+    hw, alpha, beta, ctx12, pb, xcat, gates = saved
+    f32 = dict(device=h.device, dtype=torch.float32)
+    p = _lib.ptr
+    c = lambda t: None if t is None else t.contiguous()
+    gbuf = torch.empty(B, 4 * H + 4 * D, **f32)
+    d_cell, d_h, d_cov = torch.empty(B, H, **f32), torch.empty(B, H, **f32), torch.empty(B, Lt, **f32)
+    datt, dcov_tot = torch.empty(B, Lt, **f32), torch.empty(B, Lt, **f32)
+    d_pre_b, d_ctx12 = torch.empty(2, B, D, **f32), torch.empty(2, B, D, **f32)
+    _lib.check(_lib.lib().mmb_decoder_teacher_step_bwd(
+        p(dh_head), p(g_cov), p(gates), p(cell), p(cell_out), p(c(d_h_out)), p(c(d_cell_out)), p(seq.Wcat_ctx), p(c(d_cov_out)),
+        p(alpha), p(beta), p(ctx12), p(pb), p(hw), p(seq.vb1), p(seq.vb2), p(att_cov if g_cov is not None else None),
+        p(cov_out if g_cov is not None else None), p(seq.Wb13), gbuf.data_ptr(), 4 * H + 4 * D, p(d_cell), p(datt), p(dcov_tot),
+        p(d_pre_b), p(d_ctx12), p(vec_acc), p(scal_acc), p(seq.proj_a), p(seq.proj_i), p(seq.enc_a), p(seq.enc_i), p(coverage),
+        p(seq.v1), p(seq.wc1), p(seq.v2), p(seq.wc2), p(d_proj_a), p(d_proj_i), p(d_cov), p(seq.Wh_stack), p(d_h), B, Lt, D, H, M,
+        _lib.stream()), "mmb_decoder_teacher_step_bwd")
+    _count(1)
+    return d_h, d_cell, d_cov, gbuf[:, :4 * H], d_ctx12, gbuf[:, 4 * H:], d_pre_b
 
 
 def decoder_greedy_fwd(seq: DecoderSeq, emb_text, h0, mask_u8, steps: int, target=None):
```

New measurement: 7550 (median of 6 runs). About the same (+0.2%).
